# zprodev/zlib.es

Measured on AMD Instinct MI355X. Metric: GiB/s deflate+inflate round trip, 64 MiB buffers (uncompressed bytes / wall), bit-exact vs reference, higher is better.
Workload: dtype u8; 1 GPU; random64: 1 x 64 MiB xorshift buffer(s) per GPU (seed 12345+index), deflate then inflate, HBM-resident; bytes_per_buffer=67108864, compressed_bytes=67176156, parallelism=independent buffers, one per GPU

## Files before the change

include/zes.h:

```cpp
#ifndef ZES_H
#define ZES_H

#include <stdint.h>

#ifdef __cplusplus
extern "C" {
#endif

typedef enum zes_status {
  ZES_OK = 0,
  ZES_E_NOT_DEFLATE = -1,
  ZES_E_BTYPE3 = -2,
  ZES_E_CORRUPT = -3,
  ZES_E_INSUFFICIENT = -4,
  ZES_E_LACK = -5,
  ZES_E_NOSPACE = -16,
  ZES_E_DEVICE = -17,
  ZES_E_ARG = -18,
  ZES_E_NOTRANGE = -19,
  ZES_E_GZIP = -20,
  ZES_E_CHECKSUM = -21,
  ZES_E_ZIP = -22,
  ZES_E_UNSUPPORTED = -23
} zes_status;
// ... 51 lines not shown
int zes_crc32_batch_dev(const uint8_t* d_in, const uint64_t* off, const uint64_t* len, uint32_t* crc, uint32_t count);

int zes_gzip_bound(uint64_t n, uint64_t* cap);
int zes_gzip(const uint8_t* in, uint64_t n, uint8_t* out, uint64_t cap, uint64_t* out_len);
int zes_gzip_dev(const uint8_t* d_in, uint64_t n, uint8_t* d_out, uint64_t cap, uint64_t* out_len);

#define ZES_BGZF_CHUNK 65280u
int zes_bgzip_members(uint64_t n, uint64_t* members);
int zes_bgzip_bound(uint64_t n, uint64_t* cap);
int zes_bgzip(const uint8_t* in, uint64_t n, uint8_t* out, uint64_t cap, uint64_t* out_len, uint64_t* member_off, uint32_t flags);
int zes_bgzip_dev(const uint8_t* d_in, uint64_t n, uint8_t* d_out, uint64_t cap, uint64_t* out_len, uint64_t* member_off, uint32_t flags);

int zes_gunzip(const uint8_t* in, uint64_t c, uint8_t* out, uint64_t cap, uint64_t* out_len, uint32_t flags);
int zes_gunzip_dev(const uint8_t* d_in, uint64_t c, uint8_t* d_out, uint64_t cap, uint64_t* out_len, uint32_t flags);
int zes_gunzip_alloc(const uint8_t* in, uint64_t c, zes_alloc_fn alloc, void* user, uint64_t* out_len, uint32_t flags);

int zes_bgzf_index(const uint8_t* in, uint64_t c, uint64_t* coff, uint64_t* uoff, uint64_t cap, uint64_t* members, uint32_t flags);
int zes_bgzf_index_dev(const uint8_t* d_in, uint64_t c, uint64_t* coff, uint64_t* uoff, uint64_t cap, uint64_t* members, uint32_t flags);
int zes_bgzf_read(const uint8_t* in, uint64_t c, const uint64_t* coff, const uint64_t* uoff, uint64_t members, uint64_t pos, uint64_t len,
                  uint8_t* out, uint64_t cap, uint64_t* out_len, uint32_t flags);
int zes_bgzf_read_dev(const uint8_t* d_in, uint64_t c, const uint64_t* coff, const uint64_t* uoff, uint64_t members, uint64_t pos, uint64_t len,
                      uint8_t* d_out, uint64_t cap, uint64_t* out_len, uint32_t flags);

typedef struct zes_zip_entry {
  uint64_t hdr_off;
  uint64_t name_pos;
  uint32_t csize, usize, crc;
  uint32_t name_off;
  uint16_t name_len, method, flags, pad;
} zes_zip_entry;
int zes_zip_index(const uint8_t* in, uint64_t c, zes_zip_entry* ent, uint64_t cap, uint64_t* entries, uint8_t* names, uint64_t names_cap,
                  uint64_t* names_len, uint32_t flags);
int zes_zip_index_dev(const uint8_t* d_in, uint64_t c, zes_zip_entry* ent, uint64_t cap, uint64_t* entries, uint8_t* names, uint64_t names_cap,
                      uint64_t* names_len, uint32_t flags);

int zes_zip_read_dev(const uint8_t* d_in, uint64_t c, const zes_zip_entry* ent, uint64_t nent, const uint32_t* sel, uint32_t count,
                     uint8_t* d_out, const uint64_t* out_off, uint64_t* out_len, int32_t* status, uint32_t flags);
int zes_zip_read_alloc(const uint8_t* in, uint64_t c, const zes_zip_entry* ent, uint64_t nent, const uint32_t* sel, uint32_t count,
                       zes_alloc_fn alloc, void* user, uint64_t* out_len, int32_t* status, uint32_t flags);

int zes_zipwrite_bound(const uint64_t* in_len, const uint16_t* name_len, uint32_t count, uint64_t* cap);
int zes_zipwrite_dev(const uint8_t* d_in, const uint64_t* in_off, const uint64_t* in_len, const uint8_t* names, const uint16_t* name_len,
                     uint32_t count, uint8_t* d_out, uint64_t cap, uint64_t* out_len, zes_zip_entry* ent, uint32_t flags);
int zes_zipwrite(const uint8_t* const* in, const uint64_t* in_len, const uint8_t* names, const uint16_t* name_len, uint32_t count,
                 uint8_t* out, uint64_t cap, uint64_t* out_len, zes_zip_entry* ent, uint32_t flags);

int zes_adler32(const uint8_t* in, uint64_t n, uint32_t* adler);
int zes_adler32_dev(const uint8_t* d_in, uint64_t n, uint32_t* adler);
int zes_adler32_batch_dev(const uint8_t* d_in, const uint64_t* off, const uint64_t* len, uint32_t* adler, uint32_t count);

int zes_deflate_batch_dev(const uint8_t* d_in, const uint64_t* in_off, const uint64_t* in_len,
                          uint8_t* d_out, const uint64_t* out_off, const uint64_t* out_cap,
                          uint64_t* out_len, int32_t* status, uint32_t count);
int zes_inflate_batch_dev(const uint8_t* d_in, const uint64_t* in_off, const uint64_t* in_len,
                          uint8_t* d_out, const uint64_t* out_off, const uint64_t* out_cap,
                          uint64_t* out_len, int32_t* status, uint32_t count, uint32_t flags);
int zes_deflate_batch(const uint8_t* const* in, const uint64_t* in_len, uint8_t* const* out, const uint64_t* out_cap,
                      uint64_t* out_len, int32_t* status, uint32_t count);
int zes_inflate_batch_alloc(const uint8_t* const* in, const uint64_t* in_len, zes_alloc_fn alloc, void* user,
                            uint64_t* out_len, int32_t* status, uint32_t count, uint32_t flags);

int zes_deflate_range_dev(const uint8_t* d_in, uint64_t n, uint64_t n_readable, int final_range, uint8_t* d_out, uint64_t cap,
                          uint64_t* out_bits, uint32_t* adler);
int zes_deflate_join_dev(const uint8_t* const* d_piece, const uint64_t* piece_bits, const uint32_t* piece_adler,
                         const uint64_t* piece_len, uint32_t count, uint8_t* d_out, uint64_t cap, uint64_t* out_len);

int zes_inflate_range_dev(const uint8_t* d_in, uint64_t c, uint64_t lo_bit, uint64_t own_bit, int exact_start, uint8_t* d_out,
                          uint64_t cap, uint64_t* out_len, uint64_t* first_bit, uint64_t* end_bit, uint32_t* nblocks, int* final_block);

int zes_stage_lz77_dev(const uint8_t* d_in, uint64_t n, uint64_t start, uint32_t len,
                       uint32_t* h_tokens, uint32_t* ntokens);
int zes_stage_lz77_route(uint32_t* words, uint32_t cap);
int zes_stage_huff_lengths_dev(const uint32_t* h_hist, uint32_t nsym, uint32_t maxlen, uint8_t* h_lens);
int zes_stage_chain(const uint32_t* start_bit, const uint64_t* end_bit, const uint32_t* out_len, const uint32_t* flags, uint32_t count,
                    uint32_t cap, uint32_t first_bit, int on_device, int32_t* status, uint64_t* total, uint32_t* aux, uint32_t* map);

int zes_stage_poison(uint32_t word, uint64_t* bytes);

int zes_selftest_lds_order(uint32_t iters, uint32_t seed, uint64_t* bad, uint64_t* checked);

typedef struct zes_ktime { const char* name; float ms; uint32_t launches; } zes_ktime;
int zes_last_kernel_times(zes_ktime* out, int cap);
int zes_last_inflate_tier(void);
int zes_last_gunzip_members(void);
int zes_set_profiling(int on);

int zes_gen(uint8_t* out, uint64_t n, uint32_t kind, uint32_t seed);

#ifdef __cplusplus
}
#endif
#endif
```

zlib.es_amd/__init__.py:

```python
import ctypes as C
import os
import subprocess

import numpy as np

_HERE = os.path.dirname(os.path.abspath(__file__))
_LIB_PATH = os.environ.get("ZES_LIB") or os.path.join(_HERE, "libzes_hip.so")
_lib = None

BLOCK_MAX_BUFFER_LEN = 131072

ZES_OK = 0
ZES_E_NOSPACE = -16
ZES_E_DEVICE = -17
ZES_E_ARG = -18
ZES_F_NO_FASTPATH = 1
ZES_F_LOOSE_CANDIDATES = 2
ZES_F_PIECES = 4
ZES_F_ALLOC_BOUND = 8
ZES_ALLOC_EARLY = 0x80000000
ZES_E_NOTRANGE = -19
ZES_E_GZIP = -20
ZES_E_CHECKSUM = -21
ZES_E_ZIP = -22
ZES_E_UNSUPPORTED = -23
ZES_F_GZIP_SERIAL = 32
ZES_F_INDEX_WALK = 64
ZES_F_CHECK_ADLER = 16

GEN_KINDS = {"xorshift": 0, "lowent4k": 1, "itext": 2}


class ZlibEsError(Exception):

    def __init__(self, code, message):
        super().__init__(message)
        self.code = code


class ZesKTime(C.Structure):
    _fields_ = [("name", C.c_char_p), ("ms", C.c_float), ("launches", C.c_uint32)]


ZIP_ENTRY = np.dtype([("hdr_off", "<u8"), ("name_pos", "<u8"), ("csize", "<u4"), ("usize", "<u4"), ("crc", "<u4"), ("name_off", "<u4"),
                      ("name_len", "<u2"), ("method", "<u2"), ("flags", "<u2"), ("pad", "<u2")])
assert ZIP_ENTRY.itemsize == 40

ALLOC_FN = C.CFUNCTYPE(C.c_void_p, C.c_void_p, C.c_uint32, C.c_uint64)


def build(force=False):
    srcdir = os.path.join(_HERE, "csrc")
    if force:
        subprocess.check_call(["make", "-s", "-C", srcdir, "clean"])
    subprocess.check_call(["make", "-s", "-j4", "-C", srcdir])
    return _LIB_PATH


def lib():
    global _lib
    if _lib is None:
        if not os.path.exists(_LIB_PATH):
            raise RuntimeError(
                "zlib.es_amd: %s is missing — run `python -c 'import __graft_entry__ as g; g.build()'` "
                "(there is no CPU fallback)" % _LIB_PATH)
        L = C.CDLL(_LIB_PATH)
        u64p, u32p, i32p = C.POINTER(C.c_uint64), C.POINTER(C.c_uint32), C.POINTER(C.c_int32)
        L.zes_strerror.restype = C.c_char_p
        L.zes_strerror.argtypes = [C.c_int]
        L.zes_init.argtypes = [C.c_int]
        L.zes_init_devices.argtypes = [C.c_int]
        L.zes_partition.argtypes = [C.POINTER(C.c_uint64), C.c_uint32, C.c_uint32, C.POINTER(C.c_uint32)]
        L.zes_device_info.argtypes = [C.c_char_p, C.c_int, C.POINTER(C.c_int), u64p]
        L.zes_deflate_bound.argtypes = [C.c_uint64, u64p]
        for name in ("zes_deflate", "zes_deflate_dev"):
            getattr(L, name).argtypes = [C.c_void_p, C.c_uint64, C.c_void_p, C.c_uint64, u64p]
        for name in ("zes_inflate", "zes_inflate_dev"):
            getattr(L, name).argtypes = [C.c_void_p, C.c_uint64, C.c_void_p, C.c_uint64, u64p, C.c_uint32]
        L.zes_inflate_size.argtypes = [C.c_void_p, C.c_uint64, u64p, C.c_uint32]
        L.zes_inflate_alloc.argtypes = [C.c_void_p, C.c_uint64, ALLOC_FN, C.c_void_p, u64p, C.c_uint32]
        L.zes_deflate_batch.argtypes = [C.POINTER(C.c_void_p), u64p, C.POINTER(C.c_void_p), u64p, u64p, i32p, C.c_uint32]
        L.zes_inflate_batch_alloc.argtypes = [C.POINTER(C.c_void_p), u64p, ALLOC_FN, C.c_void_p, u64p, i32p, C.c_uint32, C.c_uint32]
        L.zes_host_alloc.argtypes = [C.c_uint64, C.POINTER(C.c_void_p)]
        L.zes_host_free.argtypes = [C.c_void_p]
        for name in ("zes_deflate_raw", "zes_deflate_raw_dev"):
            getattr(L, name).argtypes = [C.c_void_p, C.c_uint64, C.c_void_p, C.c_uint64, u64p]
        for name in ("zes_inflate_raw", "zes_inflate_raw_dev"):
            getattr(L, name).argtypes = [C.c_void_p, C.c_uint64, C.c_uint64, C.c_void_p, C.c_uint64, u64p, C.c_uint32]
        for name in ("zes_inflate_raw_used", "zes_inflate_raw_used_dev"):
            getattr(L, name).argtypes = [C.c_void_p, C.c_uint64, C.c_uint64, C.c_void_p, C.c_uint64, u64p, u64p, C.c_uint32]
        for name in ("zes_crc32", "zes_crc32_dev"):
            getattr(L, name).argtypes = [C.c_void_p, C.c_uint64, u32p]
        L.zes_crc32_batch_dev.argtypes = [C.c_void_p, u64p, u64p, u32p, C.c_uint32]
        L.zes_last_gunzip_members.argtypes = []
        L.zes_gzip_bound.argtypes = [C.c_uint64, u64p]
        for name in ("zes_gzip", "zes_gzip_dev"):
            getattr(L, name).argtypes = [C.c_void_p, C.c_uint64, C.c_void_p, C.c_uint64, u64p]
        for name in ("zes_gunzip", "zes_gunzip_dev"):
            getattr(L, name).argtypes = [C.c_void_p, C.c_uint64, C.c_void_p, C.c_uint64, u64p, C.c_uint32]
        for name in ("zes_bgzip_members", "zes_bgzip_bound"):
            getattr(L, name).argtypes = [C.c_uint64, u64p]
        for name in ("zes_bgzip", "zes_bgzip_dev"):
            getattr(L, name).argtypes = [C.c_void_p, C.c_uint64, C.c_void_p, C.c_uint64, u64p, u64p, C.c_uint32]
        for name in ("zes_bgzf_index", "zes_bgzf_index_dev"):
            getattr(L, name).argtypes = [C.c_void_p, C.c_uint64, C.c_void_p, C.c_void_p, C.c_uint64, u64p, C.c_uint32]
        for name in ("zes_bgzf_read", "zes_bgzf_read_dev"):
            getattr(L, name).argtypes = [C.c_void_p, C.c_uint64, C.c_void_p, C.c_void_p, C.c_uint64, C.c_uint64, C.c_uint64, C.c_void_p, C.c_uint64,
                                         u64p, C.c_uint32]
        for name in ("zes_zip_index", "zes_zip_index_dev"):
            getattr(L, name).argtypes = [C.c_void_p, C.c_uint64, C.c_void_p, C.c_uint64, u64p, C.c_void_p, C.c_uint64, u64p, C.c_uint32]
        L.zes_zip_read_dev.argtypes = [C.c_void_p, C.c_uint64, C.c_void_p, C.c_uint64, C.c_void_p, C.c_uint32, C.c_void_p, C.c_void_p, C.c_void_p,
                                       C.c_void_p, C.c_uint32]
        L.zes_zip_read_alloc.argtypes = [C.c_void_p, C.c_uint64, C.c_void_p, C.c_uint64, C.c_void_p, C.c_uint32, ALLOC_FN, C.c_void_p, C.c_void_p,
                                         C.c_void_p, C.c_uint32]
        L.zes_zipwrite_bound.argtypes = [C.c_void_p, C.c_void_p, C.c_uint32, u64p]
        L.zes_zipwrite_dev.argtypes = [C.c_void_p, C.c_void_p, C.c_void_p, C.c_void_p, C.c_void_p, C.c_uint32, C.c_void_p, C.c_uint64, u64p, C.c_void_p,
                                       C.c_uint32]
        L.zes_zipwrite.argtypes = [C.c_void_p, C.c_void_p, C.c_void_p, C.c_void_p, C.c_uint32, C.c_void_p, C.c_uint64, u64p, C.c_void_p, C.c_uint32]
        L.zes_gunzip_alloc.argtypes = [C.c_void_p, C.c_uint64, ALLOC_FN, C.c_void_p, u64p, C.c_uint32]
        L.zes_adler32.argtypes = [C.c_void_p, C.c_uint64, u32p]
        L.zes_adler32_dev.argtypes = [C.c_void_p, C.c_uint64, u32p]
        L.zes_adler32_batch_dev.argtypes = [C.c_void_p, u64p, u64p, u32p, C.c_uint32]
        L.zes_deflate_batch_dev.argtypes = [C.c_void_p, u64p, u64p, C.c_void_p, u64p, u64p, u64p, i32p, C.c_uint32]
        L.zes_inflate_batch_dev.argtypes = [C.c_void_p, u64p, u64p, C.c_void_p, u64p, u64p, u64p, i32p, C.c_uint32,
                                            C.c_uint32]
        L.zes_deflate_range_dev.argtypes = [C.c_void_p, C.c_uint64, C.c_uint64, C.c_int, C.c_void_p, C.c_uint64, u64p, u32p]
        L.zes_inflate_range_dev.argtypes = [C.c_void_p, C.c_uint64, C.c_uint64, C.c_uint64, C.c_int, C.c_void_p, C.c_uint64, u64p, u64p, u64p,
                                            u32p, i32p]
        L.zes_deflate_join_dev.argtypes = [C.POINTER(C.c_void_p), u64p, u32p, u64p, C.c_uint32, C.c_void_p, C.c_uint64, u64p]
        L.zes_stage_lz77_dev.argtypes = [C.c_void_p, C.c_uint64, C.c_uint64, C.c_uint32, C.c_void_p, u32p]
        L.zes_stage_lz77_route.argtypes = [C.c_void_p, C.c_uint32]
        L.zes_stage_huff_lengths_dev.argtypes = [C.c_void_p, C.c_uint32, C.c_uint32, C.c_void_p]
        L.zes_stage_chain.argtypes = [u32p, u64p, u32p, u32p, C.c_uint32, C.c_uint32, C.c_uint32, C.c_int, i32p, u64p, u32p, u32p]
        L.zes_stage_poison.argtypes = [C.c_uint32, u64p]
        L.zes_selftest_lds_order.argtypes = [C.c_uint32, C.c_uint32, u64p, u64p]
        L.zes_last_kernel_times.argtypes = [C.POINTER(ZesKTime), C.c_int]
        L.zes_set_profiling.argtypes = [C.c_int]
        L.zes_pool_bytes.restype = C.c_uint64
        L.zes_pool_bytes.argtypes = []
        L.zes_gen.argtypes = [C.c_void_p, C.c_uint64, C.c_uint32, C.c_uint32]
        _lib = L
    return _lib


def strerror(code):
    return lib().zes_strerror(code).decode()


def _raise(code):
    raise ZlibEsError(code, strerror(code))


def _raise_need(rc, n):
    if rc == ZES_E_NOSPACE:
        err = ZlibEsError(rc, "%s (need %d bytes)" % (strerror(rc), n.value))
        err.need = n.value
        raise err
    if rc:
        _raise(rc)


def init(device=0):
    rc = lib().zes_init(int(device))
    if rc:
        _raise(rc)


def trim():
    rc = lib().zes_trim()
    if rc:
        _raise(rc)


def pool_bytes():
    return int(lib().zes_pool_bytes())


# ... 582 lines not shown


def _batch_call(fn, d_in, in_off, in_len, d_out, out_off, out_cap, *extra):
    import torch

    cnt = len(in_off)
    arr = lambda v: (C.c_uint64 * cnt)(*[int(x) for x in v])
    out_len = (C.c_uint64 * cnt)()
    status = (C.c_int32 * cnt)()
    torch.cuda.current_stream(d_in.device).synchronize()
    rc = fn(d_in.data_ptr(), arr(in_off), arr(in_len), d_out.data_ptr(), arr(out_off), arr(out_cap), out_len, status, cnt, *extra)
    if rc:
        _raise(rc)
    return list(out_len), list(status)


def deflate_batch_tensor(d_in, in_off, in_len, d_out, out_off, out_cap):
    return _batch_call(lib().zes_deflate_batch_dev, d_in, in_off, in_len, d_out, out_off, out_cap)


def inflate_batch_tensor(d_in, in_off, in_len, d_out, out_off, out_cap, flags=0):
    return _batch_call(lib().zes_inflate_batch_dev, d_in, in_off, in_len, d_out, out_off, out_cap, flags)


def deflate_range_tensor(t, lo, hi, final, out=None):
    import torch

    assert t.is_cuda and t.dtype == torch.uint8 and t.is_contiguous() and lo % BLOCK_MAX_BUFFER_LEN == 0
    view = _aligned(t[lo:])
    n = hi - lo
    cap = deflate_bound(n)
    if out is None:
        out = torch.empty(cap, dtype=torch.uint8, device=t.device)
    torch.cuda.current_stream(t.device).synchronize()
    bits, ad = C.c_uint64(), C.c_uint32()
    rc = lib().zes_deflate_range_dev(view.data_ptr(), n, min(view.numel(), n + 258), 1 if final else 0, out.data_ptr(), out.numel(),
                                     C.byref(bits), C.byref(ad))
    if rc:
        _raise(rc)
    return out[: (bits.value + 7) // 8], bits.value, ad.value


def deflate_join_tensors(pieces, bits, adlers, lens, out=None):
    import torch

    cnt = len(pieces)
    total = 2 + (sum(bits) + 7) // 8 + 4
    if out is None:
        out = torch.empty((total + 15) // 16 * 16, dtype=torch.uint8, device=pieces[0].device)
    torch.cuda.current_stream(out.device).synchronize()
    n = C.c_uint64()
    rc = lib().zes_deflate_join_dev((C.c_void_p * cnt)(*[p.data_ptr() for p in pieces]), (C.c_uint64 * cnt)(*bits),
                                    (C.c_uint32 * cnt)(*adlers), (C.c_uint64 * cnt)(*lens), cnt, out.data_ptr(), out.numel(), C.byref(n))
    if rc:
        _raise(rc)
    return out[: n.value]


def inflate_range_tensor(t, lo_bit, own_bit, exact, out):
    import torch

    assert t.is_cuda and t.dtype == torch.uint8 and t.is_contiguous() and out.is_cuda
    lo_bit = max(16, int(lo_bit))
    byte0 = (lo_bit >> 3) & ~15
    if byte0 >= 16:
        byte0 -= 16
    end = min(t.numel(), (int(own_bit) + 7) // 8 + (1 << 20))
    view = _aligned(t[byte0:end])
    torch.cuda.current_stream(t.device).synchronize()
    n, fb, eb, nb, fin = C.c_uint64(), C.c_uint64(), C.c_uint64(), C.c_uint32(), C.c_int32()
    rc = lib().zes_inflate_range_dev(view.data_ptr(), view.numel(), lo_bit - 8 * byte0, int(own_bit) - 8 * byte0, 1 if exact else 0,
                                     out.data_ptr(), out.numel(), C.byref(n), C.byref(fb), C.byref(eb), C.byref(nb), C.byref(fin))
    if rc == ZES_E_NOTRANGE:
        return None
    if rc:
        _raise(rc)
    return n.value, fb.value + 8 * byte0, eb.value + 8 * byte0, nb.value, bool(fin.value)


def last_inflate_tier():
    return int(lib().zes_last_inflate_tier())


def last_gunzip_members():
    return int(lib().zes_last_gunzip_members())


def set_profiling(on):
    lib().zes_set_profiling(1 if on else 0)


def last_kernel_times():
    arr = (ZesKTime * 64)()
    n = lib().zes_last_kernel_times(arr, 64)
    return [(arr[i].name.decode(), float(arr[i].ms), int(arr[i].launches)) for i in range(n)]


def stage_lz77_tensor(t, start, length):
    tok = np.empty(length + 4, dtype=np.uint32)
    nt = C.c_uint32()
    rc = lib().zes_stage_lz77_dev(t.data_ptr(), t.numel(), start, length, tok.ctypes.data, C.byref(nt))
    if rc:
        _raise(rc)
    return tok[: nt.value].copy()


def stage_lz77_route():
    w = np.zeros(9, dtype=np.uint32)
    rc = lib().zes_stage_lz77_route(w.ctypes.data, w.size)
    if rc:
        _raise(rc)
    return w


def stage_poison(word):
    n = C.c_uint64(0)
    rc = lib().zes_stage_poison(int(word) & 0xFFFFFFFF, C.byref(n))
    if rc:
        _raise(rc)
    return int(n.value)


def selftest_lds_order(iters=200, seed=1):
    bad, n = C.c_uint64(0), C.c_uint64(0)
    rc = lib().zes_selftest_lds_order(iters, seed, C.byref(bad), C.byref(n))
    if rc:
        _raise(rc)
    return int(bad.value), int(n.value)


def stage_huff_lengths(hist, maxlen):
    h = np.ascontiguousarray(hist, dtype=np.uint32)
    lens = np.zeros(h.size, dtype=np.uint8)
    rc = lib().zes_stage_huff_lengths_dev(h.ctypes.data, h.size, maxlen, lens.ctypes.data)
    if rc:
        _raise(rc)
    return lens


def stage_chain(records, cap, first_bit=16, on_device=False):
    n = len(records)
    cols = [np.ascontiguousarray([r[i] for r in records], dtype=dt) for i, dt in enumerate((np.uint32, np.uint64, np.uint32, np.uint32))]
    chain = np.zeros(max(n, 1), dtype=np.uint32)
    status, total, aux = C.c_int32(), C.c_uint64(), C.c_uint32()
    u64p, u32p = C.POINTER(C.c_uint64), C.POINTER(C.c_uint32)
    ptr = lambda a, t: a.ctypes.data_as(t) if n else None
    rc = lib().zes_stage_chain(ptr(cols[0], u32p), ptr(cols[1], u64p), ptr(cols[2], u32p), ptr(cols[3], u32p), n, int(cap), int(first_bit),
                               1 if on_device else 0, C.byref(status), C.byref(total), C.byref(aux), chain.ctypes.data_as(u32p))
    if rc:
        _raise(rc)
    return int(status.value), int(total.value), int(aux.value), [int(x) for x in chain[: aux.value]] if status.value != 1 else []
```

zlib.es_amd/csrc/zes_api.hip:

```cpp
#include "../../include/zes.h"
#include "zes_kernels.h"
#include "zes_chain.h"

#include <algorithm>
#include <atomic>
#include <condition_variable>
#include <cstdio>
#include <cstddef>
#include <cstdlib>
#include <cstring>
#include <chrono>
#include <functional>
#include <future>
#include <initializer_list>
#include <map>
#include <mutex>
#include <string>
#include <thread>
#include <vector>

extern "C" int zes_gen(uint8_t* out, uint64_t n, uint32_t kind, uint32_t seed);

namespace {

// ... 71 lines not shown
    for (const PinSpan* b = a + 1; b != s.end(); ++b)
      if (a->off < b->off + b->len && b->off < a->off + a->len) return false;
  return true;
}
#define PIN_SPAN(m) PinSpan{offsetof(PinnedArea, m), sizeof(PinnedArea::m)}
#define PIN_HOLDS(m, n) static_assert(sizeof(PinnedArea::m) >= (n), #m " is smaller than its largest user")
static_assert(sizeof(PinnedArea) <= PINNED_BYTES, "the page-locked area does not fit its allocation");
PIN_HOLDS(def.res, sizeof(ZesRes) * DEFLATE_DIRECT_BUFS);
PIN_HOLDS(def.table, sizeof(ZesBuf) * DEFLATE_TABLE_BUFS);
PIN_HOLDS(t1.counters, t1_cnt_bytes(INF_GROUP));
PIN_HOLDS(t1.res, sizeof(ZesRes) * INF_GROUP);
PIN_HOLDS(t1.table, sizeof(ZesInfBuf) * (INF_GROUP + 1));
PIN_HOLDS(t1.redo, sizeof(ZesInfBuf) * 2);
PIN_HOLDS(t1.ends, sizeof(uint64_t) * 2 * INF_GROUP);
PIN_HOLDS(first.bytes, INF_GROUP);
PIN_HOLDS(first.offs, sizeof(uint64_t) * INF_GROUP);
PIN_HOLDS(t2.search, sizeof(ZesInfBuf) * (SEG_GROUP_BUFS + 1));
PIN_HOLDS(t2.ncand, sizeof(uint32_t) * SEG_GROUP_BUFS);
PIN_HOLDS(t2.flags, sizeof(uint32_t) * (SEG_GROUP_BUFS + 1));
PIN_HOLDS(t2.res, sizeof(ZesRes) * 2 * SEG_GROUP_BUFS);
PIN_HOLDS(t2.jobs, sizeof(ZesSegJob) * SEG_GROUP_BUFS);
PIN_HOLDS(t2.live, sizeof(uint32_t) * (SEG_GROUP_BUFS + 1));
PIN_HOLDS(t2.out, sizeof(ZesSegOut) * SEG_GROUP_BUFS);
PIN_HOLDS(range[0].counters, t1_cnt_bytes(1));
PIN_HOLDS(range[0].res, sizeof(ZesRes) * 2);
static_assert(sizeof(ParMirror::cres) >= sizeof(ZesCandRes) * MIRROR_ITEMS, "the mirror is smaller than its launch bound");
static_assert(sizeof(ParMirror::start) >= sizeof(uint32_t) * MIRROR_ITEMS, "the mirror is smaller than its launch bound");
static_assert(disjoint({PIN_SPAN(range[0]), PIN_SPAN(range[1])}), "the two range slots overlap");
static_assert(disjoint({PIN_SPAN(def.res), PIN_SPAN(def.table), PIN_SPAN(crc)}), "deflate regions overlap (gzip_core: the CRC words beside the results)");
static_assert(disjoint({PIN_SPAN(t1.counters), PIN_SPAN(t1.res), PIN_SPAN(t1.table), PIN_SPAN(t1.redo), PIN_SPAN(t1.ends)}), "T1 regions overlap");
static_assert(disjoint({PIN_SPAN(first.bytes), PIN_SPAN(first.offs)}), "first-byte regions overlap");
static_assert(disjoint({PIN_SPAN(t2.search), PIN_SPAN(t2.ncand), PIN_SPAN(t2.nsurv), PIN_SPAN(t2.flags), PIN_SPAN(t2.far), PIN_SPAN(t2.res),
                        PIN_SPAN(t2.jobs), PIN_SPAN(t2.live), PIN_SPAN(t2.out)}),
              "T2 regions overlap");

#define ZES_POOLS(X)                                                                                                              \
                                                                                                             \
  X(bufs) X(blks) X(idx_a) X(idx_b) X(sdelta) X(tmask) X(mlist) X(hists) X(codes) X(hdrs) X(adler) X(res) X(order)                \
                                                                                                             \
  X(surv) X(vlong) X(segfail) X(symoff) X(cand) X(cand_sorted) X(counters) X(cres) X(map) X(resume) X(dbg) X(ibufs) X(ibufs2)     \
  X(mvlist) X(scratch) X(sres) X(maps) X(seglist) X(segprefix) X(wins) X(sym16) X(segorder) X(segjobs) X(pw16) X(gwins)           \
  X(seglive) X(segouts)                                                                                                           \
                                                                                            \
  X(st_in) X(st_out)                                                                                                              \
       \
          \
        \
            \
            \
                                                                        \
  X(crctab) X(crcacc) X(gz_in) X(gz_acc) X(gz_stage) X(gz_bodies) X(gz_outs) X(gz_tab) X(crcseg)                                  \
                  \
  X(adlerseg)

struct SurvList {
  bool ok = false;
  const uint8_t* d_in = nullptr;
  uint64_t in_off = 0, c = 0;
  uint32_t n = 0, gen = 0;
  void note(const DevBuf& list, const uint8_t* din, uint64_t off, uint64_t len, uint32_t nsurv) {
    ok = true, d_in = din, in_off = off, c = len, n = nsurv, gen = list.gen;
  }
  bool holds(const DevBuf& list, const uint8_t* din, uint64_t off, uint64_t len) const {
    return ok && gen == list.gen && list.p != nullptr && d_in == din && in_off == off && c == len;
  }
  void drop() { ok = false; }
};

struct Ctx {
  bool ready = false;
  int device = -1;
  int want = -1;
  hipStream_t stream = nullptr;
  hipStream_t cs_in = nullptr, cs_out = nullptr;
  hipEvent_t ev_up[2] = {nullptr, nullptr}, ev_k = nullptr;
  hipEvent_t ev_rng[2] = {nullptr, nullptr};
  hipStream_t s_adler = nullptr;
  hipEvent_t ev_a0 = nullptr, ev_a1 = nullptr;
#define X(name) DevBuf name;
  ZES_POOLS(X)
#undef X
  uint32_t crc_npow = 0;
  DevBuf kraft;
  PinnedArea* pinned = nullptr;
  PinnedArea* pinned_dev = nullptr;
  ParMirror* mirror = nullptr;
  ParMirror* mirror_dev = nullptr;
  ZesRes* res_more = nullptr;
  size_t res_more_n = 0;
  bool profiling = false;
  std::vector<std::pair<std::string, std::pair<hipEvent_t, hipEvent_t>>> pending;
  std::vector<hipEvent_t> event_pool;
  std::vector<std::pair<std::string, KTime>> last_times;
  std::vector<std::pair<std::string, KTime>> carry;
  std::vector<std::string> name_pool;
  int last_tier = 0;
  int last_members = 0;
  uint32_t route[ZES_ROUTE_WORDS] = {0};
  SurvList sv;
  char arch[64] = {0};
  int cus = 0;
  uint64_t hbm = 0;
};
template <class F>
void for_each_pool(Ctx& c, F fn) {
#define X(name) fn(c.name);
  ZES_POOLS(X)
#undef X
}

constexpr int ZES_MAX_DEV = 16;
Ctx g_ctx[ZES_MAX_DEV];
std::mutex g_mus[ZES_MAX_DEV];
std::atomic<int> g_nctx{1};
std::mutex g_cfg_mu;
thread_local int t_dev = 0;
thread_local bool t_routed = false;
thread_local int t_last = 0;
#define g (g_ctx[t_dev])
#define g_mu (g_mus[t_dev])
struct UseDev {
  int prev;
  bool prev_routed;
  explicit UseDev(int d) : prev(t_dev), prev_routed(t_routed) {
    if (!t_routed) t_dev = d;
    t_routed = true;
    t_last = t_dev;
  }
  ~UseDev() {
    t_dev = prev;
    t_routed = prev_routed;
  }
};

#define HIPCHK(x)                                                                              \
  do {                                                                                         \
    hipError_t e_ = (x);                                                                       \
    if (e_ != hipSuccess) {                                                                    \
      if (getenv("ZES_DEBUG")) fprintf(stderr, "zes: %s failed: %s (%s:%d)\n", #x, hipGetErrorString(e_), __FILE__, __LINE__); \
      return ZES_E_DEVICE;                                                                     \
    }                                                                                          \
  } while (0)

hipError_t release(DevBuf& b) {
  const hipError_t e = b.p ? hipFree(b.p) : hipSuccess;
  b.p = nullptr;
  b.cap = 0;
  b.gen++;
  return e;
}

int ensure(DevBuf& b, size_t bytes) {
  if (bytes <= b.cap) return ZES_OK;
  HIPCHK(release(b));
  size_t want = bytes + bytes / 8 + 4096;
  HIPCHK(hipMalloc(&b.p, want));
  b.cap = want;
  return ZES_OK;
}

int init_locked(int device) {
  if (g.ready) {
    if (device >= 0 && device != g.device) return ZES_E_ARG;
    HIPCHK(hipSetDevice(g.device));
    return ZES_OK;
  }
  int n = 0;
  if (hipGetDeviceCount(&n) != hipSuccess || n <= 0) return ZES_E_DEVICE;
  if (device < 0) device = g.want >= 0 ? g.want : 0;
  if (device >= n) return ZES_E_DEVICE;
  HIPCHK(hipSetDevice(device));
  hipDeviceProp_t prop;
  HIPCHK(hipGetDeviceProperties(&prop, device));
  snprintf(g.arch, sizeof g.arch, "%s", prop.gcnArchName);
  g.cus = prop.multiProcessorCount;
  g.hbm = prop.totalGlobalMem;
  HIPCHK(hipStreamCreateWithFlags(&g.stream, hipStreamNonBlocking));
  HIPCHK(hipStreamCreateWithFlags(&g.cs_in, hipStreamNonBlocking));
  HIPCHK(hipStreamCreateWithFlags(&g.cs_out, hipStreamNonBlocking));
  for (int k = 0; k < 2; k++) HIPCHK(hipEventCreateWithFlags(&g.ev_up[k], hipEventDisableTiming));
  for (int k = 0; k < 2; k++) HIPCHK(hipEventCreateWithFlags(&g.ev_rng[k], hipEventDisableTiming));
  HIPCHK(hipEventCreateWithFlags(&g.ev_k, hipEventDisableTiming));
  HIPCHK(hipStreamCreateWithFlags(&g.s_adler, hipStreamNonBlocking));
  HIPCHK(hipEventCreateWithFlags(&g.ev_a0, hipEventDisableTiming));
  HIPCHK(hipEventCreateWithFlags(&g.ev_a1, hipEventDisableTiming));
  auto dev_addr = [](void* h) -> void* {
    void* d = nullptr;
    if (hipHostGetDevicePointer(&d, h, 0) == hipSuccess) return d;
    (void)hipGetLastError();
    return nullptr;
  };
  HIPCHK(hipHostMalloc((void**)&g.pinned, PINNED_BYTES, hipHostMallocDefault));
  g.pinned_dev = (PinnedArea*)dev_addr(g.pinned);
  if (hipHostMalloc((void**)&g.mirror, sizeof(ParMirror), hipHostMallocDefault) == hipSuccess) {
    g.mirror_dev = (ParMirror*)dev_addr(g.mirror);
  } else {
    (void)hipGetLastError();
    g.mirror = nullptr;
  }
  {
    uint8_t tab[4096];
    for (uint32_t i = 0; i < 4096; i++) {
      uint32_t k = 0;
      for (uint32_t f = 0; f < 4; f++) k += (128u >> ((i >> (3 * f)) & 7u)) & 127u;
      tab[i] = (uint8_t)std::min(k, 200u);
    }
    HIPCHK(hipMalloc(&g.kraft.p, 4096));
    g.kraft.cap = 4096;
    HIPCHK(hipMemcpy(g.kraft.p, tab, 4096, hipMemcpyHostToDevice));
  }
  g.device = device;
  g.ready = true;
  return ZES_OK;
}

int route_host() {
  if (t_routed) return t_dev;
  const int n = g_nctx.load();
  if (n <= 1) return 0;
  static std::atomic<uint32_t> rr{0};
  return (int)(rr.fetch_add(1) % (uint32_t)n);
}
int route_dev(const void* p, const void* p2 = nullptr) {
  if (t_routed) return t_dev;
  if (g_nctx.load() <= 1 || !p) return 0;
  hipPointerAttribute_t a;
  if (hipPointerGetAttributes(&a, p) != hipSuccess) {
    (void)hipGetLastError();
    return -1;
  }
  if (p2) {
    hipPointerAttribute_t b;
    if (hipPointerGetAttributes(&b, p2) != hipSuccess) {
      (void)hipGetLastError();
      return -1;
    }
    if (b.device != a.device) return -1;
  }
  for (int i = 0, n = g_nctx.load(); i < n; i++)
    if ((g_ctx[i].ready ? g_ctx[i].device : g_ctx[i].want) == a.device) return i;
  return -1;
}
#define ROUTE_DEV(...)                    \
  const int rd_ = route_dev(__VA_ARGS__); \
  if (rd_ < 0) return ZES_E_ARG;          \
  UseDev ud(rd_)
#define LOCK_READY()                    \
  std::lock_guard<std::mutex> lk(g_mu); \
  int rc = init_locked(-1);             \
  if (rc) return rc

constexpr size_t STAGE_CHUNK = 8u << 20;
constexpr int STAGE_RING = 4;
constexpr size_t STAGE_DIRECT_MAX = 256u << 10;

struct CopyPool {
  std::vector<std::thread> threads;
  std::mutex mu;
  std::condition_variable cv_work, cv_done;
  uint8_t* dst = nullptr;
  const uint8_t* src = nullptr;
  size_t n = 0, part = 0;
  uint32_t gen = 0, parts = 0;
  std::atomic<uint32_t> next{0};
  uint32_t done = 0, active = 0;
  bool stop = false;

  void worker() {
    uint32_t seen = 0;
    std::unique_lock<std::mutex> lk(mu);
    for (;;) {
      cv_work.wait(lk, [&] { return stop || gen != seen; });
      if (stop) return;
      seen = gen;
      active++;
      lk.unlock();
      const uint32_t did = run_parts();
      lk.lock();
      done += did;
      active--;
      if (done >= parts && active == 0) cv_done.notify_all();
    }
  }
  uint32_t run_parts() {
    uint32_t did = 0;
    for (;;) {
      const uint32_t k = next.fetch_add(1);
      if (k >= parts) return did;
      const size_t o = (size_t)k * part;
      memcpy(dst + o, src + o, std::min(part, n - o));
      did++;
    }
  }
// ... 646 lines not shown

int t1_pools(uint32_t nbuf, uint32_t surv_cap, uint64_t cands, size_t counter_bytes, uint32_t nres) {
  int rc;
  if ((rc = ensure(g.ibufs, sizeof(ZesInfBuf) * (nbuf + 1)))) return rc;
  if ((rc = ensure(g.surv, (size_t)surv_cap * 8))) return rc;
  if ((rc = ensure(g.cand, (size_t)cands * 4))) return rc;
  if ((rc = ensure(g.cand_sorted, (size_t)cands * 4))) return rc;
  if ((rc = ensure(g.cres, sizeof(ZesCandRes) * cands))) return rc;
  if ((rc = ensure(g.counters, counter_bytes))) return rc;
  return ensure(g.res, sizeof(ZesRes) * nres);
}

ZesRes t1_host_chain(const uint32_t* start, const ZesCandRes* cres, const uint32_t* hc, uint32_t surv_cap, const ZesInfBuf& b, uint64_t work,
                     uint32_t* map) {
  const ZesChainView v = {start, cres, std::min(hc[4], b.cand_cap), 0u};
  const uint32_t nwork = hc[0] != 0 && hc[0] <= surv_cap ? (uint32_t)std::min<uint64_t>(v.n, work) : 0u;
  return zes_chain_decide(v, hc[4], b.cand_cap, nwork, 16u + (uint64_t)b.start_rel, map);
}

struct T1Group {
  const uint8_t* d_in;
  uint8_t* d_out;
  InfJob* jobs;
  const uint32_t* ids;
  uint32_t nbuf, flags;
  bool check_first, one;
  ZesInfBuf* hb;
  uint32_t* hc;
  ZesRes* hres;
  uint64_t chunks = 0, cands = 0, total_c = 0, work = 0;
  uint32_t surv_cap = 0;
  size_t cnt_bytes = 0;
  const ZesInfBuf* dbufs = nullptr;
  uint32_t *counters = nullptr, *cnt = nullptr;
  unsigned long long* dbg = nullptr;
  bool hostchain = false;
  std::vector<uint32_t> ncand;
  std::vector<ZesRes> r1;
};
constexpr int T1_OVER = 1;

bool t1_first_byte(T1Group& t, uint32_t i, uint8_t fb) {
  InfJob& j = t.jobs[t.ids[i]];
  if (fb & 0x40u) j.btype0 = (fb >> 4) & 3;
  if (!t.check_first || (fb & 15u) == 8u) return false;
  j.status = ZES_E_NOT_DEFLATE;
  j.tier = -1;
  return true;
}

int t1_table(T1Group& t) {
  int rc;
  g.sv.drop();
  ZesInfBuf* hb = t.hb;
  for (uint32_t i = 0; i < t.nbuf; i++) {
    const InfJob& j = t.jobs[t.ids[i]];
    ZesInfBuf& b = hb[i] = inf_buf(j);
    b.first_chunk = (uint32_t)t.chunks;
    b.cand_base = (uint32_t)t.cands;
    b.cand_cap = (uint32_t)std::min<uint64_t>(j.c / 64 + 64, j.cap / ZES_BLK + 65);
    b.own_rel = 0xFFFFFFFFu;
    t.chunks += (j.c + INF_SCAN_BYTES - 1) / INF_SCAN_BYTES;
    t.cands += b.cand_cap;
    t.total_c += j.c;
  }
  if (t.chunks >= (1ull << 31) || t.cands >= (1ull << 31)) return T1_OVER;
  const uint32_t nbuf = t.nbuf;
  memset(&hb[nbuf], 0, sizeof(ZesInfBuf));
  hb[nbuf].first_chunk = (uint32_t)t.chunks;
  hb[nbuf].cand_base = (uint32_t)t.cands;
  if (t.one) {
    hb[1].work_first = ZES_WORK_AUTO;
    hb[1].cand_cap = hb[0].cand_cap;
  }
  t.surv_cap = (uint32_t)std::min<uint64_t>(t.total_c / 4 + 1024ull * nbuf, 1ull << 30);
  t.cnt_bytes = t1_cnt_bytes(nbuf);
  if ((rc = t1_pools(nbuf, t.surv_cap, t.cands, t.cnt_bytes, nbuf))) return rc;
  if ((rc = ensure(g.map, (size_t)t.cands * 4))) return rc;
  t.dbufs = (const ZesInfBuf*)g.ibufs.p;
  t.counters = (uint32_t*)g.counters.p;
  t.cnt = t.counters + 4;
  if (t.one) {
    hipLaunchKernelGGL(k_inf_set_table1, dim3(1), dim3(64), 0, g.stream, hb[0], hb[1], (ZesInfBuf*)g.ibufs.p, t.counters,
                       (uint32_t)(t.cnt_bytes / 4));
  } else {
    HIPCHK(hipMemcpyAsync(g.ibufs.p, hb, sizeof(ZesInfBuf) * (nbuf + 1), hipMemcpyHostToDevice, g.stream));
    HIPCHK(hipMemsetAsync(g.counters.p, 0, t.cnt_bytes, g.stream));
  }
  return ZES_OK;
}

int t1_decode(T1Group& t) {
  int rc;
  const uint32_t nbuf = t.nbuf;
  ZesInfBuf* hb = t.hb;
  uint32_t* hc = t.hc;
  if (!t.one) {
    HIPCHK(hipMemcpyAsync(hc, g.counters.p, t.cnt_bytes, hipMemcpyDeviceToHost, g.stream));
    HIPCHK(hipStreamSynchronize(g.stream));
    const uint8_t* hfirst = (const uint8_t*)(hc + 4 + nbuf);
    for (uint32_t i = 0; i < nbuf; i++)
      if (t1_first_byte(t, i, hfirst[i])) hc[4 + i] = 0;
    const uint32_t nsurv0 = hc[0];
    if (nsurv0 != 0 && nsurv0 <= t.surv_cap)
      for (uint32_t i = 0; i < nbuf; i++) {
        t.ncand[i] = hc[4 + i];
        hb[i].work_first = (uint32_t)t.work;
        if (t.ncand[i] > 0 && t.ncand[i] <= hb[i].cand_cap) t.work += t.ncand[i];
      }
    hb[nbuf].work_first = (uint32_t)t.work;
    if (t.work == 0) return T1_OVER;
    HIPCHK(hipMemcpyAsync(g.ibufs.p, hb, sizeof(ZesInfBuf) * (nbuf + 1), hipMemcpyHostToDevice, g.stream));
  } else {
    t.work = hb[1].cand_cap;
  }
  if (getenv("ZES_DEBUG_PHASES")) {
    if ((rc = ensure(g.dbg, (size_t)t.work * ZES_PAR_DBG_ROW * 8))) return rc;
    HIPCHK(hipMemsetAsync(g.dbg.p, 0, (size_t)t.work * ZES_PAR_DBG_ROW * 8, g.stream));
    t.dbg = (unsigned long long*)g.dbg.p;
  }
  uint64_t total_cap = 0;
  for (uint32_t i = 0; i < nbuf; i++) total_cap += t.jobs[t.ids[i]].cap;
  const bool two = t.total_c * 10 < total_cap * 7;
  ZesParMirror mir{};
  if (t.one && t.work <= MIRROR_ITEMS && g.mirror_dev && g.pinned_dev) {
    mir.cres_host = g.mirror_dev->cres;
    mir.start_host = g.mirror_dev->start;
    mir.counters = t.counters;
    mir.counters_host = g.pinned_dev->t1.counters;
    mir.counter_words = (uint32_t)(t.cnt_bytes / 4);
    t.hostchain = true;
  }
  launch_block_par(two ? "k_inf_block_par2" : "k_inf_block_par", two, (uint32_t)t.work, t.d_in, t.d_out, t.dbufs, nbuf, t.cnt, t.dbg, nullptr, mir);
  return ZES_OK;
}

int t1_device_chain(T1Group& t) {
  Timed tm("k_inf_chain");
  const bool direct = t.one && g.pinned_dev;
  hipLaunchKernelGGL(k_inf_chain, dim3(t.nbuf), dim3(256), 0, g.stream, t.dbufs, (const uint32_t*)t.cnt, (const uint32_t*)g.cand_sorted.p,
                     (const ZesCandRes*)g.cres.p, (const uint32_t*)nullptr, (uint32_t*)g.map.p,
                     direct ? g.pinned_dev->t1.res : (ZesRes*)g.res.p, (const uint32_t*)t.counters, (uint32_t)(t.cnt_bytes / 4),
                     direct ? g.pinned_dev->t1.counters : (uint32_t*)nullptr);
  if (!direct) {
    if (t.one) HIPCHK(hipMemcpyAsync(t.hc, g.counters.p, t.cnt_bytes, hipMemcpyDeviceToHost, g.stream));
    HIPCHK(hipMemcpyAsync(t.hres, g.res.p, sizeof(ZesRes) * t.nbuf, hipMemcpyDeviceToHost, g.stream));
  }
  return ZES_OK;
}

int t1_verdicts(T1Group& t) {
  int rc;
  uint32_t* hc = t.hc;
  if (!t.hostchain && (rc = t1_device_chain(t))) return rc;
  host_lap("(work before the block-parallel tier)");
  HIPCHK(hipStreamSynchronize(g.stream));
  host_lap("T1: search + decode + chain");
  if (t.hostchain) {
    ZesRes r = t1_host_chain(g.mirror->start, g.mirror->cres, hc, t.surv_cap, t.hb[0], t.work, nullptr);
    if (r.status == 2) {
      if ((rc = t1_device_chain(t))) return rc;
      HIPCHK(hipStreamSynchronize(g.stream));
      r = t.hres[0];
    } else {
      t.hres[0] = r;
    }
    if (getenv("ZES_DEBUG")) {
      const ZesCandRes* hcr = g.mirror->cres;
      const uint32_t* hst = g.mirror->start;
      fprintf(stderr, "zes T1 host chain: nsurv %u cnt %u cap %u work %llu -> status %d out_len %llu | start0 %u", hc[0], hc[4], t.hb[0].cand_cap,
              (unsigned long long)t.work, r.status, (unsigned long long)r.out_len, hst[0]);
      for (uint32_t k = 0; k < std::min<uint32_t>(hc[4], 10u); k++)
        fprintf(stderr, " [%u: start %u end %llu len %u fl %u]", k, hst[k], (unsigned long long)hcr[k].end_bit, hcr[k].out_len, hcr[k].flags);
      fprintf(stderr, "\n");
    }
  }
  const uint32_t nsurv = hc[0];
  if (t.one) {
    const InfJob& j = t.jobs[t.ids[0]];
    if (t1_first_byte(t, 0, ((const uint8_t*)(hc + 5))[0])) return T1_OVER;
    t.ncand[0] = hc[4];
    if (nsurv != 0 && nsurv <= t.surv_cap && !(t.flags & ZES_F_LOOSE_CANDIDATES))
      g.sv.note(g.surv, t.d_in, j.in_off, j.c, nsurv);
    if (nsurv == 0 || nsurv > t.surv_cap || t.ncand[0] == 0 || t.ncand[0] > t.hb[0].cand_cap || t.ncand[0] > t.work) return T1_OVER;
    t.hb[0].work_first = 0;
    t.work = t.ncand[0];
  }
  t.r1.assign(t.hres, t.hres + t.nbuf);
  if (t.dbg && (rc = print_par_phases(t.dbg, t.work))) return rc;
  if (getenv("ZES_DEBUG")) {
    for (uint32_t i = 0, shown_b = 0; i < t.nbuf && shown_b < 4; i++) {
      const ZesRes& r = t.r1[i];
      if (r.status == 0) continue;
      shown_b++;
      const uint32_t nc = std::min(t.ncand[i], t.hb[i].cand_cap);
      fprintf(stderr, "zes T1: buf %u c=%llu nsurv(all)=%u ncand=%u chain status=%d aux=%u out_len=%llu\n", t.ids[i],
              (unsigned long long)t.hb[i].c, nsurv, t.ncand[i], r.status, r.aux, (unsigned long long)r.out_len);
      if (r.status != 1 || nc == 0) continue;
      std::vector<ZesCandRes> hcr(nc);
      std::vector<uint32_t> hcand(nc);
      HIPCHK(hipMemcpy(hcr.data(), (const ZesCandRes*)g.cres.p + t.hb[i].cand_base, sizeof(ZesCandRes) * nc, hipMemcpyDeviceToHost));
      HIPCHK(hipMemcpy(hcand.data(), (const uint32_t*)g.cand_sorted.p + t.hb[i].cand_base, 4 * (size_t)nc, hipMemcpyDeviceToHost));
      const ZesChainView v = {hcand.data(), hcr.data(), nc, 16u};
      int shown = 0;
      for (uint32_t k = 0; k < nc && shown < 6; k++) {
        if (k + 1 < nc ? zes_chain_link(v, hcr[k], k + 1) : (hcr[k].flags & ZES_CAND_OK) != 0) continue;
        fprintf(stderr, "  cand %u start=%u end_bit=%llu next_start=%u out_len=%u flags=%u\n", k, (uint32_t)zes_chain_start(v, k),
                (unsigned long long)hcr[k].end_bit, k + 1 < nc ? (uint32_t)zes_chain_start(v, k + 1) : 0, hcr[k].out_len, hcr[k].flags);
        shown++;
      }
    }
  }
  return ZES_OK;
}

// ... 640 lines not shown
  G.ccap.resize(nb);
  G.searched.assign(nb, 0);
  uint64_t cands = 0, max_c = 0;
  for (uint32_t k = 0; k < nb; k++) {
    const InfJob& j = G.jobs[G.ids[k]];
    G.cbase[k] = (uint32_t)cands;
    G.ccap[k] = range_cand_cap(j.c);
    cands += G.ccap[k];
    max_c = std::max(max_c, j.c);
  }
  G.surv_cap = range_surv_cap(max_c);
  G.w = seg_words(nb, nb);
  if ((rc = ensure(g.ibufs, sizeof(ZesInfBuf) * 2))) return rc;
  if ((rc = ensure(g.surv, (size_t)G.surv_cap * 8))) return rc;
  if ((rc = ensure(g.cand, (size_t)cands * 4))) return rc;
  if ((rc = ensure(g.cand_sorted, (size_t)cands * 4))) return rc;
  if ((rc = ensure(g.counters, G.w.total * 4))) return rc;
  if ((rc = ensure(g.mvlist, SEG_BUCKETS * 4))) return rc;
  G.counters = (uint32_t*)g.counters.p + G.w.scan;
  G.cnt = (uint32_t*)g.counters.p + G.w.cnt;
  G.sink = (uint8_t*)((uint32_t*)g.counters.p + G.w.sink);
  HIPCHK(hipMemsetAsync(g.counters.p, 0, G.w.total * 4, g.stream));
  G.dbufs = (const ZesInfBuf*)g.ibufs.p;
  return ZES_OK;
}

ZesInfBuf t2_search_buf(const T2Group& G, uint32_t k) {
  const InfJob& j = G.jobs[G.ids[k]];
  ZesInfBuf b = inf_buf(j);
  b.cand_base = G.cbase[k];
  b.cand_cap = G.ccap[k];
  b.start_rel = j.start0 - 16u;
  return b;
}

int t2_search_group(T2Group& G) {
  int rc;
  const uint32_t nb = G.nb;
  ZesInfBuf* hb = g.pinned->t2.search;
  uint64_t chunks = 0, total_c = 0;
  for (uint32_t k = 0; k < nb; k++) {
    hb[k] = t2_search_buf(G, k);
    hb[k].first_chunk = (uint32_t)chunks;
    chunks += (hb[k].c + INF_SCAN_BYTES - 1) / INF_SCAN_BYTES;
    total_c += hb[k].c;
  }
  memset(&hb[nb], 0, sizeof(ZesInfBuf));
  hb[nb].first_chunk = (uint32_t)chunks;
  const uint32_t surv_all = (uint32_t)std::min<uint64_t>(total_c / 4 + 1024ull * nb, 1ull << 30);
  if ((rc = ensure(g.ibufs, sizeof(ZesInfBuf) * (nb + 1)))) return rc;
  if ((rc = ensure(g.surv, (size_t)surv_all * 8))) return rc;
  G.dbufs = (const ZesInfBuf*)g.ibufs.p;
  HIPCHK(hipMemcpyAsync(g.ibufs.p, hb, sizeof(ZesInfBuf) * (nb + 1), hipMemcpyHostToDevice, g.stream));
  if ((rc = launch_search(G.d_in, G.dbufs, nb, (uint32_t)chunks, surv_all, G.counters, G.cnt, G.sink, T2_SEARCH, total_c))) return rc;
  {
    Timed t("k_inf_ranksort");
    hipLaunchKernelGGL(k_inf_ranksort, dim3(nb), dim3(1024), 0, g.stream, G.dbufs, (const uint32_t*)G.cnt, (const uint32_t*)g.cand.p,
                       (uint32_t*)g.cand_sorted.p, SEG_BUCKETS);
  }
  uint32_t* hc0 = g.pinned->t2.ncand;
  HIPCHK(hipMemcpyAsync(hc0, G.cnt, (size_t)nb * 4, hipMemcpyDeviceToHost, g.stream));
  HIPCHK(hipStreamSynchronize(g.stream));
  bool redo = false;
  for (uint32_t k = 0; k < nb; k++) {
    G.searched[k] = hc0[k] <= SEG_BUCKETS;
    redo = redo || !G.searched[k];
  }
  if (redo) {
    if ((rc = ensure(g.ibufs2, sizeof(ZesInfBuf) * 2))) return rc;
    G.dbufs = (const ZesInfBuf*)g.ibufs2.p;
  }
  return ZES_OK;
}

int t2_search_one(T2Group& G, uint32_t k) {
  int rc;
  uint32_t* cntk = G.cnt + k;
  HIPCHK(hipMemsetAsync(cntk, 0, 4, g.stream));
  const ZesInfBuf b0 = t2_search_buf(G, k);
  const uint32_t chunks = (uint32_t)((b0.c + INF_SCAN_BYTES - 1) / INF_SCAN_BYTES);
  ZesInfBuf b1;
  memset(&b1, 0, sizeof b1);
  b1.first_chunk = chunks;
  hipLaunchKernelGGL(k_inf_set_table1, dim3(1), dim3(64), 0, g.stream, b0, b1, const_cast<ZesInfBuf*>(G.dbufs), G.counters, 4u);
  const bool reuse = G.nb == 1 && g.sv.holds(g.surv, G.d_in, b0.in_off, b0.c) && b0.start_rel == 0u && g.sv.n <= G.surv_cap;
  g.sv.drop();
  if (reuse) {
    g.pinned->t2.nsurv = g.sv.n;
    HIPCHK(hipMemcpyAsync(G.counters, &g.pinned->t2.nsurv, 4, hipMemcpyHostToDevice, g.stream));
    rc = launch_verify(G.d_in, G.dbufs, G.surv_cap, G.counters, cntk, T2_SEARCH.loose, b0.c);
  } else {
    rc = launch_search(G.d_in, G.dbufs, 1u, chunks, G.surv_cap, G.counters, cntk, G.sink, T2_SEARCH, b0.c);
  }
  if (rc) return rc;
  Timed t("k_inf_cand_thin");
  const uint32_t bucket_bits = (uint32_t)((b0.c * 8 + SEG_BUCKETS - 1) / SEG_BUCKETS);
  HIPCHK(hipMemsetAsync(g.mvlist.p, 0xFF, SEG_BUCKETS * 4, g.stream));
  hipLaunchKernelGGL(k_inf_cand_bucket, dim3((uint32_t)std::min<uint64_t>(b0.cand_cap / 256 + 1, 1024)), dim3(256), 0, g.stream,
                     (const uint32_t*)g.cand.p + b0.cand_base, (const uint32_t*)cntk, b0.cand_cap, bucket_bits, (uint32_t*)g.mvlist.p);
  hipLaunchKernelGGL(k_inf_cand_compact, dim3(1), dim3(1024), 0, g.stream, (const uint32_t*)g.mvlist.p,
                     (uint32_t*)g.cand_sorted.p + b0.cand_base, cntk);
  return ZES_OK;
}

int t2_group_counts(T2Group& G) {
  const uint32_t nb = G.nb;
  uint32_t* hc = g.pinned->t2.ncand;
  HIPCHK(hipMemcpyAsync(hc, G.cnt, (size_t)nb * 4, hipMemcpyDeviceToHost, g.stream));
  host_lap("(host work since)");
  HIPCHK(hipStreamSynchronize(g.stream));
  host_lap("T2: search (verify, thinning)");
  G.nc.assign(hc, hc + nb);
  if (getenv("ZES_T2_DBG")) {
    for (uint32_t k = 0; k < nb; k++) {
      std::vector<uint32_t> hcand(std::min<uint32_t>(G.nc[k], SEG_BUCKETS));
      if (!hcand.empty()) HIPCHK(hipMemcpy(hcand.data(), (const uint32_t*)g.cand_sorted.p + G.cbase[k], hcand.size() * 4, hipMemcpyDeviceToHost));
      fprintf(stderr, "zes T2 candidates buf %u (%zu):", k, hcand.size());
      for (uint32_t v : hcand) fprintf(stderr, " %u", v + 16u);
      fprintf(stderr, "\n");
    }
  }
  return ZES_OK;
}

int t2_group_runs(T2Group& G) {
  int rc;
  std::vector<uint32_t> rid, rbase, rn;
  for (uint32_t k = 0; k < G.nb;) {
    uint32_t work = 0;
    rid.clear();
    rbase.clear();
    rn.clear();
    for (; k < G.nb; k++) {
      if (G.nc[k] > SEG_BUCKETS) continue;
      if (!rid.empty() && work + G.nc[k] + 1 > SEG_GROUP_WORK) break;
      rid.push_back(G.ids[k]);
      rbase.push_back(G.cbase[k]);
      rn.push_back(G.nc[k]);
      work += G.nc[k] + 1;
    }
    const uint32_t nr = (uint32_t)rid.size();
    if (nr && (rc = inflate_segments_run(G.d_in, G.d_out, G.jobs, rid.data(), rbase.data(), rn.data(), nr, seg_words(G.nb, nr)))) return rc;
  }
  return ZES_OK;
}

int inflate_segments(const uint8_t* d_in, uint8_t* d_out, InfJob* jobs, const std::vector<uint32_t>& all) {
  int rc;
  for (size_t g0 = 0; g0 < all.size(); g0 += SEG_GROUP_BUFS) {
    T2Group G{d_in, d_out, jobs, all.data() + g0, (uint32_t)std::min<size_t>(SEG_GROUP_BUFS, all.size() - g0)};
    if ((rc = t2_group_table(G))) return rc;
    if (G.nb > 1 && (rc = t2_search_group(G))) return rc;
    for (uint32_t k = 0; k < G.nb; k++)
      if (!G.searched[k] && (rc = t2_search_one(G, k))) return rc;
    if ((rc = t2_group_counts(G))) return rc;
    if ((rc = t2_group_runs(G))) return rc;
  }
  return ZES_OK;
}

constexpr uint64_t STORED_MIN_C = 65536;
int inflate_segments_pieces(const uint8_t* d_in, uint8_t* d_out, InfJob& j) {
  static const uint64_t piece = [] {
    const char* e = getenv("ZES_SEG_PIECE_MB");
    const uint64_t mb = e ? strtoull(e, nullptr, 10) : 0;
    return mb ? (mb << 20) : (32ull << 20);
  }();
// ... 19 lines not shown
    }
    if (sub[0].tier != 2) return ZES_OK;
    piece_now = piece;
    if (sub[0].status == ZES_E_NOSPACE) nospace = true;
    else if (sub[0].status != ZES_OK) return ZES_OK;
    out_base += sub[0].out_len;
    if (sub[0].final_seen) {
      j.tier = 2;
      j.status = (nospace || out_base > j.cap) ? ZES_E_NOSPACE : ZES_OK;
      j.out_len = out_base;
      j.end_bit = 8 * byte0 + sub[0].end_bit;
      return ZES_OK;
    }
    const uint64_t next_bit = 8 * byte0 + sub[0].end_bit;
    if (!sub[0].partial || next_bit <= pos_bit) return ZES_OK;
    pos_bit = next_bit;
  }
  return ZES_OK;
}

int inflate_stored(const uint8_t* d_in, uint8_t* d_out, InfJob& j) {
  int rc;
  const uint64_t cap_entries = std::min<uint64_t>(j.c / 5 + 1, 1ull << 22);
  if ((rc = ensure(g.res, sizeof(ZesRes)))) return rc;
  if ((rc = ensure(g.scratch, (size_t)cap_entries * sizeof(ZesStoredBlk)))) return rc;
  ZesRes hr;
  hr.status = 1;
  constexpr uint64_t STORED_PAR_MAX_C = 128ull << 20;
  constexpr uint32_t STORED_CHUNK_H = 16384, STORED_SLOTS_H = 8;
  if (j.c >= (2ull << 20) && j.c <= STORED_PAR_MAX_C && !getenv("ZES_NO_STORED_PAR")) {
    const uint32_t nchunks = (uint32_t)((j.c + STORED_CHUNK_H - 1) / STORED_CHUNK_H);
    if ((rc = ensure(g.mvlist, (size_t)nchunks * (STORED_SLOTS_H + 1) * 4))) return rc;
    uint32_t* slots = (uint32_t*)g.mvlist.p;
    uint32_t* counts = slots + (size_t)nchunks * STORED_SLOTS_H;
    {
      Timed t("k_inf_stored_find");
      hipLaunchKernelGGL(k_inf_stored_find, dim3(nchunks), dim3(256), 0, g.stream, d_in, j.in_off, (uint32_t)j.c, slots, counts);
    }
    {
      Timed t("k_inf_stored_rank");
      hipLaunchKernelGGL(k_inf_stored_rank, dim3(1), dim3(1024), 0, g.stream, d_in, j.in_off, (uint32_t)j.c, (const uint32_t*)slots,
                         (const uint32_t*)counts, nchunks, cap_entries, (ZesStoredBlk*)g.scratch.p, (ZesRes*)g.res.p);
    }
    if ((rc = read_res(&hr))) return rc;
  }
  if (hr.status != 0) {
    Timed t("k_inf_stored_walk");
    hipLaunchKernelGGL(k_inf_stored_walk, dim3(1), dim3(64), 0, g.stream, d_in, j.in_off, j.c, cap_entries, (ZesStoredBlk*)g.scratch.p,
                       (ZesRes*)g.res.p);
    if ((rc = read_res(&hr))) return rc;
  }
  if (hr.status != 0) return ZES_OK;
  j.tier = 2;
  j.out_len = hr.out_len;
  j.status = hr.out_len > j.cap ? ZES_E_NOSPACE : ZES_OK;
  if (j.want_end && hr.aux) {
    ZesStoredBlk last;
    HIPCHK(hipMemcpy(&last, (const ZesStoredBlk*)g.scratch.p + hr.aux - 1, sizeof last, hipMemcpyDeviceToHost));
    j.end_bit = 8 * (last.src + last.len);
  }
  if (j.status == ZES_OK && hr.aux) {
    Timed t("k_inf_stored_copy");
    hipLaunchKernelGGL(k_inf_stored_copy, dim3(hr.aux), dim3(256), 0, g.stream, d_in, j.in_off, d_out, j.out_off, (const ZesStoredBlk*)g.scratch.p);
    HIPCHK(hipStreamSynchronize(g.stream));
  }
  return ZES_OK;
}

int inflate_slow(const uint8_t* d_in, uint8_t* d_out, InfJob& j) {
  int rc;
  if ((rc = ensure(g.res, 2 * sizeof(ZesRes)))) return rc;
  if ((rc = ensure(g.resume, 16))) return rc;
  ZesRes hr;
  bool have_resume = false;
  if (j.c >= 3) {
#ifdef WD_PROFILE
    if ((rc = ensure(g.dbg, 64))) return rc;
    HIPCHK(hipMemsetAsync(g.dbg.p, 0, 64, g.stream));
    zes_wd_set_dbg((unsigned long long*)g.dbg.p);
#endif
    {
      const ZesInfBuf b0 = inf_buf(j);
      if ((rc = ensure(g.ibufs, sizeof(ZesInfBuf) * 2))) return rc;
      hipLaunchKernelGGL(k_inf_set_table1, dim3(1), dim3(64), 0, g.stream, b0, b0, (ZesInfBuf*)g.ibufs.p, (uint32_t*)nullptr, 0u);
      Timed t("k_inf_decode_seq");
      hipLaunchKernelGGL(k_inf_decode, dim3(1), dim3(64), 0, g.stream, d_in, d_out, (const ZesInfBuf*)g.ibufs.p, (ZesRes*)g.res.p,
                         (uint64_t*)g.resume.p);
    }
    if ((rc = read_res(&hr))) return rc;
#ifdef WD_PROFILE
    {
      unsigned long long h[8];
      HIPCHK(hipMemcpy(h, g.dbg.p, 64, hipMemcpyDeviceToHost));
      const double n = (double)std::max<unsigned long long>(h[5], 1);
      fprintf(stderr, "zes wave decoder: %llu tokens, cycles per token: lit/len entry %.1f, literal path %.1f, distance entry %.1f, copy %.1f, flush test %.1f; kernel %.1f\n",
              h[5], h[0] / n, h[1] / n, h[2] / n, h[3] / n, h[4] / n, h[6] / n);
    }
#endif
    if (hr.status == 0) {
      j.tier = 3;
      j.out_len = hr.out_len;
      j.status = hr.out_len > j.cap ? ZES_E_NOSPACE : ZES_OK;
      if (j.want_end) HIPCHK(hipMemcpy(&j.end_bit, g.resume.p, 8, hipMemcpyDeviceToHost));
      return ZES_OK;
    }
    have_resume = true;
  }
  {
    Timed t("k_inf_exact");
    hipLaunchKernelGGL(k_inf_exact, dim3(1), dim3(64), 0, g.stream, d_in, j.in_off, j.c, d_out, j.out_off, j.cap,
                       have_resume ? (const uint64_t*)g.resume.p : (const uint64_t*)nullptr, (ZesRes*)g.res.p);
  }
  if ((rc = read_res(&hr))) return rc;
  if (j.want_end) {
    ZesRes r2;
    HIPCHK(hipMemcpy(&r2, (const ZesRes*)g.res.p + 1, sizeof r2, hipMemcpyDeviceToHost));
    j.end_bit = r2.out_len;
  }
  j.tier = 4;
  j.out_len = hr.out_len;
  j.status = hr.status;
  return ZES_OK;
}

constexpr uint64_t T1_PIECE = 256ull << 20;
constexpr uint64_t T1_PIECE_SLACK = 1ull << 20;
int inflate_pieces(const uint8_t* d_in, uint8_t* d_out, InfJob& j, uint32_t flags) {
  uint64_t piece = T1_PIECE;
  if (flags & ZES_F_PIECES) piece = 1ull << 20;
  uint64_t pos_bit = 16, total = 0, blocks = 0;
  for (uint32_t round = 0; round < (1u << 20); round++) {
    uint64_t byte0 = (pos_bit >> 3) & ~15ull;
    if (byte0 >= 16) byte0 -= 16;
    const uint64_t rel = pos_bit - 8 * byte0;
    const uint64_t pc = std::min<uint64_t>(j.c - byte0, piece + T1_PIECE_SLACK);
    const uint64_t done_bytes = blocks * ZES_BLK;
    RangeRes rr;
    int rc = inflate_t1_range(d_in, j.in_off + byte0, pc, rel, rel + piece * 8, true, d_out, j.out_off + std::min(done_bytes, j.cap),
                              j.cap > done_bytes ? j.cap - done_bytes : 0, flags, &rr);
    if (rc) return rc;
    if (!rr.handled || rr.nblocks == 0) return ZES_OK;
    blocks += rr.nblocks;
    total += rr.out_len;
    pos_bit = 8 * byte0 + rr.end_bit;
    if (rr.final_block) {
      j.tier = 1;
      j.out_len = total;
      j.end_bit = pos_bit;
      j.status = total > j.cap ? ZES_E_NOSPACE : ZES_OK;
      return ZES_OK;
    }
    if (pos_bit >= j.c * 8) return ZES_OK;
  }
  return ZES_OK;
}

int gather_bytes(const uint8_t* d_in, const std::vector<InfJob>& jobs, const uint32_t* ids, uint32_t nb, uint32_t at, const uint8_t** bytes) {
  int rc;
  if ((rc = ensure(g.ibufs, (size_t)INF_GROUP * 8 + INF_GROUP))) return rc;
  uint64_t* ho = g.pinned->first.offs;
  for (uint32_t k = 0; k < nb; k++) ho[k] = jobs[ids[k]].in_off + at;
  uint8_t* dfirst = (uint8_t*)g.ibufs.p + (size_t)INF_GROUP * 8;
  HIPCHK(hipMemcpyAsync(g.ibufs.p, ho, (size_t)nb * 8, hipMemcpyHostToDevice, g.stream));
  hipLaunchKernelGGL(k_inf_first_bytes, dim3((nb + 255) / 256), dim3(256), 0, g.stream, d_in, (const uint64_t*)g.ibufs.p, dfirst, nb);
  HIPCHK(hipMemcpyAsync(g.pinned->first.bytes, dfirst, nb, hipMemcpyDeviceToHost, g.stream));
  HIPCHK(hipStreamSynchronize(g.stream));
  *bytes = g.pinned->first.bytes;
// ... 286 lines not shown
    case ZES_E_CORRUPT: return "Data is corrupted";
    case ZES_E_INSUFFICIENT: return "Data length is insufficient";
    case ZES_E_LACK: return "Lack of data length";
    case ZES_E_NOSPACE: return "zes: output capacity too small";
    case ZES_E_DEVICE: return "zes: HIP device error (no gfx950 device or runtime failure)";
    case ZES_E_ARG: return "zes: bad argument";
    case ZES_E_NOTRANGE: return "zes: not a clean chain of reference-made blocks in this range";
    case ZES_E_GZIP: return "zes: not a valid gzip member (header or trailer)";
    case ZES_E_CHECKSUM: return "zes: checksum mismatch";
    case ZES_E_ZIP: return "zes: not a valid ZIP archive or entry (end record, directory or local header)";
    case ZES_E_UNSUPPORTED: return "zes: unsupported ZIP feature (ZIP64, several disks, encryption, a method other than 0 or 8)";
    default: return "zes: unknown status";
  }
}

int zes_init(int device) {
  UseDev ud(0);
  std::lock_guard<std::mutex> lk(g_mu);
  return init_locked(device);
}

int zes_init_devices(int n) {
  int have = 0;
  if (hipGetDeviceCount(&have) != hipSuccess || have <= 0) return ZES_E_DEVICE;
  const bool over = getenv("ZES_OVERSUBSCRIBE") != nullptr;
  if (n <= 0) n = have;
  if (n > ZES_MAX_DEV || (n > have && !over)) return ZES_E_ARG;
  std::lock_guard<std::mutex> cfg(g_cfg_mu);
  for (int i = 0; i < n; i++) {
    std::lock_guard<std::mutex> lk(g_mus[i]);
    const int dev = i % have;
    if (g_ctx[i].ready ? g_ctx[i].device != dev : (g_ctx[i].want >= 0 && g_ctx[i].want != dev)) return ZES_E_ARG;
    g_ctx[i].want = dev;
  }
  if (n > g_nctx.load()) g_nctx.store(n);
  for (int i = 0; i < n; i++) {
    UseDev ud(i);
    LOCK_READY();
  }
  return ZES_OK;
}

static int shutdown_one(void);
int zes_shutdown(void) {
  std::lock_guard<std::mutex> cfg(g_cfg_mu);
  int rc = ZES_OK;
  for (int i = 0; i < ZES_MAX_DEV; i++) {
    t_dev = i;
    const int r = shutdown_one();
    if (r && !rc) rc = r;
    g_ctx[i].want = -1;
  }
  t_dev = 0;
  g_nctx.store(1);
  return rc;
}

static void free_scratch_locked() {
  for_each_pool(g, [](DevBuf& b) { (void)release(b); });
}

int zes_trim(void) {
  std::lock_guard<std::mutex> cfg(g_cfg_mu);
  const int keep = t_dev;
  for (int i = 0; i < ZES_MAX_DEV; i++) {
    t_dev = i;
    std::lock_guard<std::mutex> lk(g_mu);
    if (!g.ready) continue;
    (void)hipSetDevice(g.device);
    (void)hipStreamSynchronize(g.stream);
    free_scratch_locked();
  }
  t_dev = keep;
  return ZES_OK;
}

static int shutdown_one(void) {
  std::lock_guard<std::mutex> lk(g_mu);
  if (!g.ready) return ZES_OK;
  (void)hipSetDevice(g.device);
  (void)hipStreamSynchronize(g.stream);
  free_scratch_locked();
  (void)release(g.kraft);
  if (g.pinned) (void)hipHostFree(g.pinned);
  if (g.mirror) (void)hipHostFree(g.mirror);
  if (g.res_more) (void)hipHostFree(g.res_more);
  g.pinned = g.pinned_dev = nullptr;
  g.mirror = g.mirror_dev = nullptr;
  g.res_more = nullptr;
  g.res_more_n = 0;
  g_side_up.shutdown();
  g_side_down.shutdown();
  g_up.release();
  g_down.release();
  for (hipEvent_t e : g.event_pool) (void)hipEventDestroy(e);
  g.event_pool.clear();
  (void)hipStreamDestroy(g.stream);
  (void)hipStreamDestroy(g.cs_in);
  (void)hipStreamDestroy(g.cs_out);
  for (int k = 0; k < 2; k++) (void)hipEventDestroy(g.ev_up[k]);
  for (int k = 0; k < 2; k++) (void)hipEventDestroy(g.ev_rng[k]);
  (void)hipEventDestroy(g.ev_k);
  (void)hipStreamDestroy(g.s_adler);
  (void)hipEventDestroy(g.ev_a0);
  (void)hipEventDestroy(g.ev_a1);
  g.s_adler = nullptr;
  g.stream = g.cs_in = g.cs_out = nullptr;
  g.ready = false;
  return ZES_OK;
}

int zes_host_alloc(uint64_t n, void** p) {
  UseDev ud(0);
  if (!p) return ZES_E_ARG;
  *p = nullptr;
  LOCK_READY();
  HIPCHK(hipHostMalloc(p, n ? n : 1, hipHostMallocPortable));
  return ZES_OK;
}

int zes_host_free(void* p) {
  if (!p) return ZES_OK;
  std::lock_guard<std::mutex> lk(g_mu);
  if (g.ready) (void)hipSetDevice(g.device);
  HIPCHK(hipHostFree(p));
  return ZES_OK;
}

int zes_device_info(char* name, int cap, int* cus, uint64_t* hbm_bytes) {
  LOCK_READY();
  if (name && cap > 0) snprintf(name, (size_t)cap, "%s", g.arch);
  if (cus) *cus = g.cus;
  if (hbm_bytes) *hbm_bytes = g.hbm;
  return ZES_OK;
}

int zes_deflate_bound(uint64_t n, uint64_t* cap) {
  if (!cap) return ZES_E_ARG;
  *cap = deflate_bound(n);
  return ZES_OK;
}

int zes_deflate_batch_dev(const uint8_t* d_in, const uint64_t* in_off, const uint64_t* in_len, uint8_t* d_out,
                          const uint64_t* out_off, const uint64_t* out_cap, uint64_t* out_len, int32_t* status, uint32_t count) {
  ROUTE_DEV(d_in, d_out);
  if (!in_off || !in_len || !out_off || !out_cap || !out_len || !status) return ZES_E_ARG;
  LOCK_READY();
  return deflate_batch_core(d_in, in_off, in_len, d_out, out_off, out_cap, out_len, status, count);
}

int zes_deflate_dev(const uint8_t* d_in, uint64_t n, uint8_t* d_out, uint64_t cap, uint64_t* out_len) {
  ROUTE_DEV(d_in, d_out);
  if (!out_len) return ZES_E_ARG;
  uint64_t zero = 0;
  int32_t st = 0;
  int rc = zes_deflate_batch_dev(d_in, &zero, &n, d_out, &zero, &cap, out_len, &st, 1);
  return rc ? rc : st;
}

struct SettleGuard {
  std::future<int>&a, &b;
  ~SettleGuard() {
    if (a.valid()) a.wait();
    if (b.valid()) b.wait();
  }
};
// ... 2318 lines not shown
    if ((rc = t1_pools(1, 0, (uint64_t)cap + 1, sizeof hc, 1))) return rc;
    if ((rc = ensure(g.map, (size_t)cap * 4 + 4))) return rc;
    uint32_t* counters = (uint32_t*)g.counters.p;
    HIPCHK(hipMemcpyAsync(g.ibufs.p, tab, sizeof tab, hipMemcpyHostToDevice, g.stream));
    HIPCHK(hipMemcpyAsync(counters, hc, sizeof hc, hipMemcpyHostToDevice, g.stream));
    if (n) {
      HIPCHK(hipMemcpyAsync(g.cand_sorted.p, rel.data(), (size_t)n * 4, hipMemcpyHostToDevice, g.stream));
      HIPCHK(hipMemcpyAsync(g.cres.p, cres.data(), sizeof(ZesCandRes) * n, hipMemcpyHostToDevice, g.stream));
    }
    hipLaunchKernelGGL(k_inf_chain, dim3(1), dim3(256), 0, g.stream, (const ZesInfBuf*)g.ibufs.p, (const uint32_t*)(counters + 4),
                       (const uint32_t*)g.cand_sorted.p, (const ZesCandRes*)g.cres.p, (const uint32_t*)nullptr, (uint32_t*)g.map.p, (ZesRes*)g.res.p,
                       (const uint32_t*)counters, 0u, (uint32_t*)nullptr);
    HIPCHK(hipGetLastError());
    if ((rc = read_res(&r))) return rc;
    if (r.status != 1 && r.aux <= n) HIPCHK(hipMemcpy(map, g.map.p, (size_t)r.aux * 4, hipMemcpyDeviceToHost));
  }
  *status = r.status;
  *total = r.out_len;
  *aux = r.aux;
  return ZES_OK;
}

static int poison_locked(Ctx& c, uint32_t word, uint64_t* filled) {
  HIPCHK(hipSetDevice(c.device));
  const hipStream_t streams[] = {c.stream, c.cs_in, c.cs_out, c.s_adler};
  for (hipStream_t s : streams) HIPCHK(hipStreamSynchronize(s));
  hipError_t e = hipSuccess;
  for_each_pool(c, [&](DevBuf& b) {
    const size_t words = b.p ? b.cap / 4 : 0;
    if (!words || e != hipSuccess) return;
    e = hipMemsetD32Async((hipDeviceptr_t)b.p, (int)word, words, c.stream);
    *filled += (uint64_t)words * 4;
  });
  HIPCHK(e);
  auto fill = [&](void* p, size_t bytes) {
    if (!p) return;
    std::fill((uint32_t*)p, (uint32_t*)p + bytes / 4, word);
    *filled += bytes / 4 * 4;
  };
  fill(c.pinned, PINNED_BYTES);
  fill(c.mirror, sizeof(ParMirror));
  fill(c.res_more, sizeof(ZesRes) * c.res_more_n);
  c.sv.drop();
  c.crc_npow = 0;
  HIPCHK(hipStreamSynchronize(c.stream));
  return ZES_OK;
}

int zes_stage_poison(uint32_t word, uint64_t* bytes) {
  std::lock_guard<std::mutex> cfg(g_cfg_mu);
  uint64_t filled = 0;
  int rc = ZES_OK;
  for (int i = 0; i < ZES_MAX_DEV; i++) {
    std::lock_guard<std::mutex> lk(g_mus[i]);
    if (!g_ctx[i].ready) continue;
    const int r = poison_locked(g_ctx[i], word, &filled);
    if (r && !rc) rc = r;
  }
  if (bytes) *bytes = filled;
  return rc;
}

int zes_selftest_lds_order(uint32_t iters, uint32_t seed, uint64_t* bad, uint64_t* checked) {
  if (!bad || !checked || iters == 0 || iters > 100000u) return ZES_E_ARG;
  LOCK_READY();
  if ((rc = ensure(g.hists, 320 * 4))) return rc;
  HIPCHK(hipMemsetAsync(g.hists.p, 0, 16, g.stream));
  hipLaunchKernelGGL(k_selftest_lds_order, dim3(256), dim3(SORT_THREADS), 0, g.stream, (unsigned long long*)g.hists.p, iters, seed);
  HIPCHK(hipGetLastError());
  unsigned long long h[2] = {0, 0};
  HIPCHK(hipMemcpyAsync(h, g.hists.p, 16, hipMemcpyDeviceToHost, g.stream));
  HIPCHK(hipStreamSynchronize(g.stream));
  *bad = h[0];
  *checked = h[1];
  return ZES_OK;
}

int zes_last_inflate_tier(void) {
  UseDev ud(t_last);
  std::lock_guard<std::mutex> lk(g_mu);
  return g.last_tier;
}

int zes_last_gunzip_members(void) {
  UseDev ud(t_last);
  std::lock_guard<std::mutex> lk(g_mu);
  return g.last_members;
}

int zes_set_profiling(int on) {
  std::lock_guard<std::mutex> cfg(g_cfg_mu);
  for (int i = 0; i < ZES_MAX_DEV; i++) {
    std::lock_guard<std::mutex> lk(g_mus[i]);
    g_ctx[i].profiling = on != 0;
  }
  return ZES_OK;
}

uint64_t zes_pool_bytes(void) {
  uint64_t total = 0;
  for (int i = 0; i < ZES_MAX_DEV; i++) {
    std::lock_guard<std::mutex> lk(g_mus[i]);
    for_each_pool(g_ctx[i], [&](const DevBuf& b) { total += b.cap; });
  }
  return total;
}

int zes_last_kernel_times(zes_ktime* out, int cap) {
  UseDev ud(t_last);
  std::lock_guard<std::mutex> lk(g_mu);
  int n = 0;
  g.name_pool.clear();
  for (auto& e : g.last_times) g.name_pool.push_back(e.first);
  for (size_t i = 0; i < g.last_times.size() && n < cap; i++, n++) {
    out[n].name = g.name_pool[i].c_str();
    out[n].ms = (float)g.last_times[i].second.ms;
    out[n].launches = g.last_times[i].second.launches;
  }
  return n;
}

}
```

zlib.es_amd/csrc/zes_inflate.hip:

```cpp
#include "zes_common.h"
#include "zes_kernels.h"
#include "zes_chain.h"

#define ZES_E_NOT_DEFLATE (-1)
#define ZES_E_BTYPE3 (-2)
#define ZES_E_CORRUPT (-3)
#define ZES_E_INSUFFICIENT (-4)
#define ZES_E_LACK (-5)

__device__ static inline uint64_t g_load64_le(const uint8_t* p, uint64_t byte, uint64_t nbytes) {
  uint64_t v = 0;
#pragma unroll
  for (int k = 0; k < 8; k++) {
    const uint64_t b = byte + k;
    v |= (uint64_t)(b < nbytes ? p[b] : (uint8_t)0) << (8 * k);
  }
  return v;
}

#define SCAN_BYTES INF_SCAN_BYTES
#define RANK_LDS 8192u
#define VERIFY_STEPS 32u
#define SCAN_LIST 1024u
__global__ __launch_bounds__(256) void k_inf_move_slots(uint8_t* __restrict__ dst, const uint8_t* __restrict__ src,
                                                        const uint32_t* __restrict__ dst_slot, const uint32_t* __restrict__ src_slot,
                                                        uint32_t nitems) {
  const uint32_t item = blockIdx.x >> 5, part = blockIdx.x & 31u;
  if (item >= nitems) return;
  const uint4* s4 = reinterpret_cast<const uint4*>(src + (uint64_t)src_slot[item] * ZES_BLK) + part * 256u;
  uint4* d4 = reinterpret_cast<uint4*>(dst + (uint64_t)dst_slot[item] * ZES_BLK) + part * 256u;
  d4[threadIdx.x] = s4[threadIdx.x];
}

__global__ void k_inf_set_table1(ZesInfBuf b0, ZesInfBuf sentinel, ZesInfBuf* __restrict__ bufs, uint32_t* __restrict__ counters,
                                 uint32_t nwords) {
  if (threadIdx.x == 0) {
    bufs[0] = b0;
    bufs[1] = sentinel;
  }
  if (counters && threadIdx.x < nwords) counters[threadIdx.x] = 0;
}

__global__ void k_inf_set_table_range(ZesInfBuf b0, ZesInfBuf sentinel, ZesInfBuf* __restrict__ bufs, uint32_t* __restrict__ counters,
                                      uint32_t nwords, const unsigned long long* __restrict__ acc, unsigned long long dcap) {
  if (threadIdx.x == 0) {
    const unsigned long long off = acc[0] * ZES_BLK;
    b0.out_off += off < dcap ? off : dcap;
    b0.cap = dcap - (off < dcap ? off : dcap);
    bufs[0] = b0;
    bufs[1] = sentinel;
  }
  if (counters && threadIdx.x < nwords) counters[threadIdx.x] = 0;
}

__global__ void k_inf_first_bytes(const uint8_t* __restrict__ d_in, const uint64_t* __restrict__ offs, uint8_t* __restrict__ out,
                                  uint32_t n) {
  const uint32_t i = blockIdx.x * blockDim.x + threadIdx.x;
  if (i < n) out[i] = d_in[offs[i]];
}

__device__ __forceinline__ static uint32_t buf_of_chunk(const ZesInfBuf* bufs, uint32_t nbuf, uint32_t x) {
  uint32_t lo = 0, hi = nbuf;
  while (hi - lo > 1) {
    const uint32_t mid = (lo + hi) >> 1;
    if (bufs[mid].first_chunk <= x) lo = mid; else hi = mid;
  }
  return lo;
}

#define SCAN_FINAL_ZONE_BITS (160u * 1024u * 8u)
__global__ __launch_bounds__(INF_SCAN_THREADS) void k_inf_scan(const uint8_t* __restrict__ d_in, const ZesInfBuf* __restrict__ bufs,
                                                               uint32_t nbuf, unsigned long long* __restrict__ surv,
                                                               uint32_t surv_cap, uint32_t* __restrict__ counters,
                                                               uint8_t* __restrict__ first_bytes, uint32_t mode,
                                                               const uint8_t* __restrict__ kraft_tab) {
  const uint32_t loose = mode & 1u;
  __shared__ __align__(16) uint32_t s[SCAN_BYTES / 4 + 8];
  __shared__ uint32_t s_list[SCAN_LIST];
  __shared__ uint32_t s_cnt, s_base;
  __shared__ __align__(16) uint8_t s_kraft[4096];
  const uint32_t tid = threadIdx.x;
  if (tid == 0) s_cnt = 0;
  static_assert(INF_SCAN_THREADS * 16 == 4096, "one 16-byte load per thread");
  reinterpret_cast<uint4*>(s_kraft)[tid] = reinterpret_cast<const uint4*>(kraft_tab)[tid];
  const uint32_t bi = buf_of_chunk(bufs, nbuf, blockIdx.x);
  const uint64_t in_off = bufs[bi].in_off, c = bufs[bi].c;
  const uint64_t b0 = (uint64_t)(blockIdx.x - bufs[bi].first_chunk) * SCAN_BYTES;
  const uint32_t* in32 = reinterpret_cast<const uint32_t*>(d_in + in_off);
  const uint64_t ndw = (c + 3) >> 2;
  uint32_t hdr2 = 0;
  bool hdr_known = false;
  if ((mode & 2u) && !loose && !(bufs[bi].range_flags & ZES_START_ANY)) {
    const uint64_t hbit = 16ull + bufs[bi].start_rel;
    if (hbit + 3 <= c * 8) {
      const uint64_t hb = hbit >> 3;
      hdr2 = ((uint32_t)d_in[in_off + hb] | ((uint32_t)d_in[in_off + (hb + 1 < c ? hb + 1 : hb)] << 8)) >> (uint32_t)(hbit & 7u);
      hdr_known = true;
    }
  }
  {
    constexpr uint32_t NLD = (SCAN_BYTES / 4 + 8 + INF_SCAN_THREADS - 1) / INF_SCAN_THREADS;
    uint32_t v[NLD];
#pragma unroll
    for (uint32_t j = 0; j < NLD; j++) {
      const uint64_t gi = (b0 >> 2) + tid + j * INF_SCAN_THREADS;
      v[j] = in32[gi < ndw ? gi : ndw - 1];
    }
#pragma unroll
    for (uint32_t j = 0; j < NLD; j++) {
      const uint32_t i = tid + j * INF_SCAN_THREADS;
      const uint64_t gi = (b0 >> 2) + i;
      uint32_t x = v[j];
      if (gi == ndw - 1 && (c & 3u)) x &= (1u << (8u * (uint32_t)(c & 3u))) - 1u;
      if (gi >= ndw) x = 0;
      if (i < SCAN_BYTES / 4 + 8) s[i] = x;
    }
  }
  __syncthreads();
  if (tid == 0 && b0 == 0) first_bytes[bi] = (uint8_t)((s[0] & 0x0fu) | (((s[0] >> 17) & 3u) << 4) | 0x40u);
  if (hdr_known && ((hdr2 >> 1) & 3u) != 2u) return;
  const uint64_t end_bits = c * 8;
// ... 2538 lines not shown
```

zlib.es_amd/csrc/zes_inflate_par.hip:

```cpp
#include "zes_common.h"
#include "zes_kernels.h"
#include "zes_chain.h"

#define PL_ROOT 10u
#define PD_ROOT 9u
#define F_EOB 1u
#define F_FAIL 2u
#define F_VOID 4u
#define F_HIST 8u

#define RES_W 4096u
#define P4_SPARSE_DEP_MAX 32u
#define P4_SPARSE_MAX 1024u
#ifndef RES_REPS
#define RES_REPS 4u
#endif
#define PAR_CHUNK (ZES_BLK - 3u * RES_W)
#define PAR_DIST_OFF (PAR_CHUNK + 64u)
#define PAR_MAX_OUT (1u << 27)
#define STAGE_DW ((ZES_BLK + ZES_BLK / 8) / 4)
struct ParSmem {
  uint8_t out[ZES_BLK];
  uint32_t bitmap[ZES_BLK / 32];
  uint32_t lut_l[1u << PL_ROOT];
// ... 87 lines not shown

struct Lit8 {
  uint32_t lo, n, off;
};
__device__ __forceinline__ static uint32_t lead_lit8(uint32_t w, const Lit8& f) {
  const uint32_t r = __brev(w);
  const bool a = ((r >> 24) - f.lo) < f.n, b = (((r >> 16) & 255u) - f.lo) < f.n, c = (((r >> 8) & 255u) - f.lo) < f.n,
             d = ((r & 255u) - f.lo) < f.n;
  uint32_t n = d ? 4u : 3u;
  n = c ? n : 2u;
  n = b ? n : 1u;
  n = a ? n : 0u;
  return n;
}

struct SegTab {
  uint64_t a, b, c, d, e, f, g, h;
};
__device__ __forceinline__ static uint32_t tab_get(const SegTab& t, uint32_t o) {
  const uint32_t wi = o >> 3;
  uint64_t a = t.a, b = t.b, c = t.c, d = t.d, e = t.e, f = t.f, g = t.g, h = t.h;
  asm("" : "+v"(a), "+v"(b), "+v"(c), "+v"(d));
  asm("" : "+v"(e), "+v"(f), "+v"(g), "+v"(h));
  uint64_t x = a;
  x = (wi == 1u) ? b : x;
  x = (wi == 2u) ? c : x;
  x = (wi == 3u) ? d : x;
  x = (wi == 4u) ? e : x;
  x = (wi == 5u) ? f : x;
  x = (wi == 6u) ? g : x;
  x = (wi == 7u) ? h : x;
  return (uint32_t)(x >> ((o & 7u) * 8u)) & 0xffu;
}
__device__ __forceinline__ static void tab_set(SegTab& t, uint32_t o, uint32_t code) {
  const uint32_t wi = o >> 3;
  const uint64_t v = (uint64_t)code << ((o & 7u) * 8u);
  t.a |= (wi == 0u) ? v : 0ull;
  t.b |= (wi == 1u) ? v : 0ull;
  t.c |= (wi == 2u) ? v : 0ull;
  t.d |= (wi == 3u) ? v : 0ull;
  t.e |= (wi == 4u) ? v : 0ull;
  t.f |= (wi == 5u) ? v : 0ull;
  t.g |= (wi == 6u) ? v : 0ull;
  t.h |= (wi == 7u) ? v : 0ull;
}
__device__ __forceinline__ static void tab_put(SegTab& t, uint32_t o, uint32_t code, bool doit) {
  const uint32_t wi = o >> 3, sh = (o & 7u) * 8u;
  const uint64_t m = doit ? (0xffull << sh) : 0ull, v = doit ? ((uint64_t)code << sh) : 0ull;
  t.a = (wi == 0u) ? ((t.a & ~m) | v) : t.a;
  t.b = (wi == 1u) ? ((t.b & ~m) | v) : t.b;
  t.c = (wi == 2u) ? ((t.c & ~m) | v) : t.c;
  t.d = (wi == 3u) ? ((t.d & ~m) | v) : t.d;
  t.e = (wi == 4u) ? ((t.e & ~m) | v) : t.e;
  t.f = (wi == 5u) ? ((t.f & ~m) | v) : t.f;
  t.g = (wi == 6u) ? ((t.g & ~m) | v) : t.g;
  t.h = (wi == 7u) ? ((t.h & ~m) | v) : t.h;
}
__device__ __forceinline__ static uint64_t tab_nzmask(const SegTab& t) {
  auto nz8 = [](uint64_t w) -> uint64_t {
    const uint64_t k7 = 0x7f7f7f7f7f7f7f7full;
    const uint64_t y = (((w & k7) + k7) | w) & ~k7;
    return ((y >> 7) * 0x0102040810204080ull) >> 56;
  };
  return nz8(t.a) | (nz8(t.b) << 8) | (nz8(t.c) << 16) | (nz8(t.d) << 24) | (nz8(t.e) << 32) | (nz8(t.f) << 40) | (nz8(t.g) << 48) | (nz8(t.h) << 56);
}
__device__ __forceinline__ static uint64_t bcast64(uint64_t v, uint32_t srclane) {
  const uint32_t lo = (uint32_t)__builtin_amdgcn_readlane((int)(uint32_t)v, (int)srclane);
  const uint32_t hi = (uint32_t)__builtin_amdgcn_readlane((int)(uint32_t)(v >> 32), (int)srclane);
  return (uint64_t)lo | ((uint64_t)hi << 32);
}
__device__ __forceinline__ static SegTab tab_bcast(const SegTab& t, uint32_t srclane) {
  SegTab r;
  r.a = bcast64(t.a, srclane);
  r.b = bcast64(t.b, srclane);
  r.c = bcast64(t.c, srclane);
  r.d = bcast64(t.d, srclane);
  r.e = bcast64(t.e, srclane);
  r.f = bcast64(t.f, srclane);
  r.g = bcast64(t.g, srclane);
  r.h = bcast64(t.h, srclane);
  return r;
}

__device__ __forceinline__ static int slow_sym(const LaneBits& b, uint32_t root, const uint16_t* syms, const uint32_t* first,
                                               const uint16_t* cnt, const uint16_t* offs, uint32_t* len_out) {
  uint32_t code = __brev((uint32_t)b.bb & ((1u << root) - 1u)) >> (32u - root);
  for (uint32_t len = root + 1; len <= 15u; len++) {
    code = (code << 1) | (uint32_t)((b.bb >> (len - 1)) & 1u);
    const uint32_t f = first[len];
    const uint32_t rel = code - f;
    if (code >= f && rel < cnt[len]) {
      *len_out = len;
      return (int)syms[offs[len] + rel];
    }
  }
  return -1;
}

#define T_LIT 0u
#define T_EOB 1u
#define T_MATCH 2u
#define T_FAIL 3u
#define C_EOB 62u
#define C_FAIL 63u
#define C_NONE 255u

template <bool LDS>
__device__ __forceinline__ static uint32_t tok_step(ParSmem& S, LaneBits& b, const BitSrc& src, uint32_t& val, uint32_t& len,
                                                    uint32_t& dist) {
  lb_refill<LDS>(b, src);
  uint32_t e = S.lut_l[(uint32_t)b.bb & ((1u << PL_ROOT) - 1u)];
  if ((e & 15u) == 0u) {
    uint32_t l2 = 0;
    const int sy = slow_sym(b, PL_ROOT, S.syms_l, S.first_l, S.cnt_l, S.offs_l, &l2);
    if (sy < 0) return T_FAIL;
    e = entry_l((uint32_t)sy, l2);
  }
  lb_take(b, e & 15u);
  const uint32_t kind = (e >> 8) & 3u;
  if (kind == 0u) {
    val = e >> 16;
    return T_LIT;
  }
  if (kind == 1u) return T_EOB;
  if (kind == 3u) return T_FAIL;
  lb_refill<LDS>(b, src);
  len = (e >> 16) + lb_take(b, (e >> 4) & 15u);
  lb_refill<LDS>(b, src);
  uint32_t ed = S.lut_d[(uint32_t)b.bb & ((1u << PD_ROOT) - 1u)];
  if ((ed & 15u) == 0u) {
    uint32_t l2 = 0;
    const int sy = slow_sym(b, PD_ROOT, S.syms_d, S.first_d, S.cnt_d, S.offs_d, &l2);
    if (sy < 0) return T_FAIL;
    ed = entry_d((uint32_t)sy, l2);
  }
  lb_take(b, ed & 15u);
  if (((ed >> 8) & 3u) != 2u) return T_FAIL;
  lb_refill<LDS>(b, src);
  dist = (ed >> 16) + lb_take(b, (ed >> 4) & 15u);
  return T_MATCH;
}

__device__ __forceinline__ static uint32_t lut_l_entry(ParSmem& S, uint32_t bits) {
  uint32_t e = S.lut_l[bits & ((1u << PL_ROOT) - 1u)];
  if ((e & 15u) == 0u) {
    LaneBits t;
    t.bb = bits;
    uint32_t l2 = 0;
    const int sy = slow_sym(t, PL_ROOT, S.syms_l, S.first_l, S.cnt_l, S.offs_l, &l2);
    e = sy < 0 ? 0u : entry_l((uint32_t)sy, l2);
  }
  return e;
}
__device__ __forceinline__ static uint32_t lut_d_entry(ParSmem& S, uint32_t bits) {
  uint32_t e = S.lut_d[bits & ((1u << PD_ROOT) - 1u)];
  if ((e & 15u) == 0u) {
    LaneBits t;
    t.bb = bits;
    uint32_t l2 = 0;
    const int sy = slow_sym(t, PD_ROOT, S.syms_d, S.first_d, S.cnt_d, S.offs_d, &l2);
    e = sy < 0 ? 0u : entry_d((uint32_t)sy, l2);
  }
  return e;
}

__device__ __forceinline__ static void lb_refill_bf(LaneBits& b, const BitSrc& s) {
  const bool need = b.nb <= 32u;
  const uint32_t k = ((b.pos + b.nb) >> 5) - s.s_first;
  const bool in = k < s.s_count;
  const uint32_t kk = in ? k : 0u;
  uint32_t w = s.s32[kk ^ ((kk >> 5) & 31u)];
  w = in ? w : 0u;
  const uint32_t sh = need ? b.nb : 0u;
  const uint64_t add = (uint64_t)w << sh;
  b.bb |= need ? add : 0ull;
  b.nb += need ? 32u : 0u;
}

__device__ __forceinline__ static void len_step(ParSmem& S, const BitSrc& src, LaneBits& b, bool act, uint32_t& adv, bool& eob,
                                                bool& bad) {
  lb_refill_bf(b, src);
  const uint32_t a = S.len_l[(uint32_t)b.bb & ((1u << PL_ROOT) - 1u)];
  uint32_t n = a & 63u;
  const bool sp = (a & 0x80u) != 0u;
  bool m = (a & 0x40u) != 0u;
  eob = false;
  bad = false;
  if (__ballot(act && sp)) {
    const uint32_t e = lut_l_entry(S, (uint32_t)b.bb);
    const uint32_t kind = (e >> 8) & 3u;
    if (sp) {
      eob = kind == 1u;
      bad = (kind == 3u) || ((e & 15u) == 0u);
      n = (e & 15u) + ((e >> 4) & 15u);
      m = kind == 2u;
    }
  }
  if (__ballot(act && m)) {
    LaneBits t = b;
    t.bb >>= n;
    t.nb -= n;
    t.pos += n;
    lb_refill_bf(t, src);
    const uint32_t d = S.len_d[(uint32_t)t.bb & ((1u << PD_ROOT) - 1u)];
    uint32_t n2 = d & 63u;
    const bool dsp = (d & 0x80u) != 0u;
    if (__ballot(act && m && dsp)) {
      const uint32_t ed = lut_d_entry(S, (uint32_t)t.bb);
      if (dsp) {
        bad = bad || (m && ((((ed >> 8) & 3u) != 2u) || (ed & 15u) == 0u));
        n2 = (ed & 15u) + ((ed >> 4) & 15u);
      }
    }
    if (act && m) {
      b = t;
      n = n2;
    }
  }
  adv = n;
}

#define NX_EOB 0xFEu
#define NX_FAIL 0xFFu

__device__ __forceinline__ static uint32_t win_bits(uint32_t a0, uint32_t a1, uint32_t a2, uint32_t a3, uint32_t a4, uint32_t r) {
  const uint32_t wi = r >> 5;
  uint32_t lo = a0, hi = a1;
  lo = (wi == 1u) ? a1 : lo;
  hi = (wi == 1u) ? a2 : hi;
  lo = (wi == 2u) ? a2 : lo;
  hi = (wi == 2u) ? a3 : hi;
  lo = (wi == 3u) ? a3 : lo;
  hi = (wi == 3u) ? a4 : hi;
  return __builtin_amdgcn_alignbit(hi, lo, r & 31u);
}

#define F8_MAXSEG 1800u
#define F8_LIST 32u

__device__ __forceinline__ static bool seg_table_f8(ParSmem& S, const BitSrc& src, uint32_t limit, uint32_t base, uint32_t stop,
                                                    const Lit8& f8, SegTab& tab, unsigned long long* dp) {
#define T8STAMP(i)                                                                  \
  do {                                                                              \
// ... 591 lines not shown
        const uint32_t adv = 8u * nlit;
        ob += nlit;
        b.bb >>= adv;
        b.nb -= adv;
        b.pos += adv;
      }
    }
    if (act && b.pos >= stop) act = false;
    lb_refill<LDS>(b, src);
    const uint32_t e = lut_l_entry(S, (uint32_t)b.bb);
    const uint32_t kind = (e >> 8) & 3u;
    const uint32_t cl = e & 15u, xb = (e >> 4) & 15u;
    uint32_t adv = cl + xb;
    bool bad = (kind == 3u) || (cl == 0u);
    uint32_t len = (e >> 16) + (((uint32_t)(b.bb >> cl)) & ((1u << xb) - 1u));
    uint32_t dist = 0;
    const bool ismatch = act && kind == 2u;
    if (__ballot(ismatch)) {
      LaneBits t = b;
      t.bb >>= adv;
      t.nb -= adv;
      t.pos += adv;
      lb_refill<LDS>(t, src);
      const uint32_t ed = lut_d_entry(S, (uint32_t)t.bb);
      const uint32_t dl = ed & 15u, dx = (ed >> 4) & 15u;
      dist = (ed >> 16) + (((uint32_t)(t.bb >> dl)) & ((1u << dx) - 1u));
      bad = bad || (kind == 2u && ((((ed >> 8) & 3u) != 2u) || dl == 0u));
      if (ismatch) {
        b = t;
        adv = dl + dx;
      }
    }
    adv = act ? adv : 0u;
    b.bb >>= adv;
    b.nb -= adv;
    b.pos += adv;
    if (act && (bad || b.pos > limit)) {
      fl |= F_FAIL;
      act = false;
    }
    if (act && kind == 1u) {
      fl |= F_EOB;
      act = false;
    }
    if (act) {
      if (kind == 0u) {
        if (ACC) {
          put((e >> 16) & 255u, 1u);
        } else if (EMIT) {
          const uint32_t q = out_off + ob - clo;
          if (!HIST || q < PAR_CHUNK) S.out[q] = (uint8_t)(e >> 16);
        }
        ob += 1u;
      } else {
        if (ACC) flush();
        if (EMIT) {
          const uint32_t p = out_off + ob, q = p - clo;
          if (!HIST && dist > p) {
            fl |= F_HIST;
          } else if (!HIST || q < PAR_CHUNK) {
            S.out[q] = (uint8_t)(dist - 1u);
            S.out[q + 1] = (uint8_t)((dist - 1u) >> 8);
            S.out[q + 2] = (uint8_t)(len - 3u);
            atomicOr(&S.bitmap[q >> 5], 1u << (q & 31u));
          } else if (p < clo && p + len > clo) {
            S.res_strad[0] = p + len - clo;
            S.res_strad[1] = dist;
          }
        }
        ob += len;
      }
      if (ob > (HIST ? PAR_MAX_OUT : ZES_BLK)) {
        fl |= F_FAIL;
        act = false;
      }
    }
  }
  if (ACC) flush();
  exit_pos = b.pos;
  outbytes = ob;
  flags = fl;
}

__device__ __forceinline__ static bool par_build(ParSmem& S, uint32_t base, uint32_t nsym, uint32_t chunk, bool is_dist, uint16_t* syms, uint32_t* first,
                                                 uint16_t* cnt, uint16_t* offs) {
  const uint32_t lane = zes_lane();
  const uint8_t* lens = S.lens + base;
  uint32_t c[16], before[16];
#pragma unroll
  for (int l = 0; l < 16; l++) c[l] = before[l] = 0;
  uint32_t myl = 0;
  for (uint32_t s0 = 0; s0 < nsym; s0 += 64) {
    const uint32_t s = s0 + lane;
    const uint32_t l = s < nsym ? lens[s] : 0u;
    if (s0 == 64u * chunk) {
      myl = l;
#pragma unroll
      for (int k = 1; k < 16; k++) before[k] = c[k];
    }
#pragma unroll
    for (int k = 1; k < 16; k++) c[k] += (uint32_t)__popcll(__ballot(l == (uint32_t)k));
  }
  uint32_t code = 0, off = 0, kraft = 0;
  uint32_t fst[16], ofs[16];
#pragma unroll
  for (int l = 1; l < 16; l++) {
    fst[l] = code;
    ofs[l] = off;
    code = (code + c[l]) << 1;
    off += c[l];
    kraft += c[l] << (15 - l);
  }
  if (kraft > 32768u) return false;
  if (chunk == 0u) {
    if (!is_dist) {
      uint32_t n8 = 0;
      for (uint32_t s0 = 0; s0 < 256u; s0 += 64) n8 += (uint32_t)__popcll(__ballot(lens[s0 + lane] == 8u));
      if (lane == 0) {
        S.f8lo = fst[8];
        S.f8n = n8 >= 128u ? n8 : 0u;
        S.f8off = ofs[8];
      }
    }
    if (lane < 16) {
      uint32_t f = 0, o2 = 0, cc = 0;
#pragma unroll
      for (int l = 1; l < 16; l++)
        if ((int)lane == l) {
          f = fst[l];
          o2 = ofs[l];
          cc = c[l];
        }
      first[lane] = f;
      offs[lane] = (uint16_t)o2;
      cnt[lane] = (uint16_t)cc;
    }
  }
  uint64_t same = ~0ull;
#pragma unroll
  for (int bt = 0; bt < 4; bt++) {
    const bool bit = (myl >> bt) & 1u;
    const uint64_t bal = __ballot(bit);
    same &= bit ? bal : ~bal;
  }
  if (myl) {
    uint32_t o2 = 0;
#pragma unroll
    for (int k = 1; k < 16; k++)
      if ((int)myl == k) o2 = ofs[k] + before[k];
    syms[o2 + (uint32_t)__popcll(same & zes_lanemask_lt())] = (uint16_t)(64u * chunk + lane);
  }
  return true;
}
template <uint32_t ROOT, bool IS_DIST>
__device__ __forceinline__ static void par_fill(uint32_t i, const uint16_t* syms, const uint32_t* first, const uint16_t* cnt, const uint16_t* offs,
                                                uint32_t* lut, uint8_t* blut) {
  uint32_t fst[ROOT + 1], cn[ROOT + 1], ofs[ROOT + 1];
#pragma unroll
  for (uint32_t l = 1; l <= ROOT; l++) {
    fst[l] = first[l];
    cn[l] = cnt[l];
    ofs[l] = offs[l];
  }
  const uint32_t msb = __brev(i) >> (32u - ROOT);
  uint32_t at = 0, len = 0;
#pragma unroll
// ... 180 lines not shown
    if (bad && lane == 0) atomicOr(&S.status, 1u);
    if (!past && !bad) {
      uint64_t m = 0;
      uint32_t cur = en, nsym = 0;
      while (cur < 64u) {
        const uint32_t v = (uint32_t)__builtin_amdgcn_readlane((int)pk, (int)cur);
        m |= 1ull << cur;
        nsym++;
        cur = v & 127u;
      }
      asm volatile("s_waitcnt lgkmcnt(0)" ::: "memory");
      if ((m >> lane) & 1ull) s_cl[(uint32_t)__popcll(m & zes_lanemask_lt())] = pk;
      asm volatile("s_waitcnt lgkmcnt(0)" ::: "memory");
      const uint32_t tc = s_cl[lane];
      const bool on = lane < nsym;
      const uint32_t s1 = on ? (tc >> 15) & 31u : 0u, r1 = on ? (tc >> 7) & 255u : 0u;
      const bool hole = on && !((tc >> 20) & 1u);
      const uint32_t is16 = (uint32_t)(on && !hole && s1 == 16u);
      const uint32_t valraw = s1 >= 16u ? 0u : s1;
      const uint32_t srcl = ph_scan_max((on && !is16) ? lane + 1u : 0u);
      const uint32_t vsrc = (uint32_t)__builtin_amdgcn_ds_bpermute((int)((srcl ? srcl - 1u : 0u) << 2), (int)valraw);
      const uint32_t val = srcl ? vsrc : prev;
      const uint32_t kin = ph_scan_add(r1);
      const uint32_t kk = k + kin - r1;
      const uint64_t endm = __ballot(on && !hole && kk + r1 >= total);
      const uint32_t cut = endm ? (uint32_t)__builtin_ctzll(endm) : nsym - 1u;
      const bool mine = on && lane <= cut;
      const uint64_t badm = __ballot(mine && (hole || (is16 && kk == 0u) || kk + r1 > total));
      if (badm) {
        if (lane == 0) atomicOr(&S.status, 1u);
      } else {
        if (mine && val) {
          for (uint32_t q = 0; q < r1; q++) {
            const uint32_t idx = kk + q;
            S.lens[idx < HLIT ? idx : 288 + (idx - HLIT)] = (uint8_t)val;
          }
        }
        if (endm) {
          const uint32_t nx = (uint32_t)__builtin_amdgcn_readlane((int)(tc & 127u), (int)cut);
          if (lane == 0) {
            S.hdr_end = wb + nx;
            S.h_done = 1;
          }
        } else if (wave == PAR_WAVES - 1u && lane == 0) {
          S.h_off = cur - 64u;
          S.h_k = (uint32_t)__builtin_amdgcn_readlane((int)(kk + r1), (int)cut);
          S.h_prev = (uint32_t)__builtin_amdgcn_readlane((int)val, (int)cut);
        }
      }
    }
    __syncthreads();
    if (S.status || S.h_done) break;
    off0 = S.h_off;
    k0 = S.h_k;
    prev0 = S.h_prev;
    wbase0 += 64u * PAR_WAVES;
    __syncthreads();
  }
  if (wave == 0) HSTAMP(2);
  if (!S.status && S.hdr_end > limit && threadIdx.x == 0) S.status = 1;
}

struct ParItem {
  const uint32_t* g32;
  uint32_t lastdw, limit, start;
  uint32_t de_est, de_est2;
  ZesCandRes* cres;
  ZesCandRes* cres_host;
  uint32_t* start_host;
  uint8_t* dst;
  uint64_t room;
  ZesSegRes* sres;
  uint32_t* sym;
  uint64_t sym_cap;
  uint32_t* sym_all;
  unsigned long long* bump;
  uint64_t bump_base, bump_cap;
  uint64_t* symoff;
  uint32_t* map;
  const uint32_t* cand;
  uint32_t ncand;
  uint32_t* fail_list;
  uint32_t w;
};

template <bool FOREIGN, bool TWO>
__device__ __forceinline__ static void par_body(ParSmem& S, const ParItem& it, unsigned long long* dbg) {
#define STAMP(i)                                                     \
  do {                                                               \
    if (dbg && threadIdx.x == 0) dbg[(size_t)blockIdx.x * ZES_PAR_DBG_ROW + (i)] = (unsigned long long)clock64(); \
  } while (0)
#define PAR_DECLINE(END_BIT, TOTAL)                                   \
  do {                                                                \
    if (threadIdx.x == 0) {                                           \
      if (FOREIGN) {                                                  \
        ZesSegRes r_;                                                 \
        r_.end_bit = 0;                                               \
        r_.out_len = 0;                                               \
        r_.flags = 0;                                                 \
        r_.next = 0;                                                  \
        *it.sres = r_;                                                \
        it.fail_list[1u + atomicAdd(&it.fail_list[0], 1u)] = it.w;    \
      } else {                                                        \
        ZesCandRes r_;                                                \
        r_.end_bit = (END_BIT);                                       \
        r_.out_len = (TOTAL);                                         \
        r_.flags = 0;                                                 \
        *it.cres = r_;                                                \
        if (it.cres_host) {                                           \
          *it.cres_host = r_;                                         \
          *it.start_host = it.start;                                  \
        }                                                             \
      }                                                               \
    }                                                                 \
  } while (0)
  const uint32_t tid = threadIdx.x, lane = tid & 63u, wave = tid >> 6;
  const uint32_t lastdw = it.lastdw, limit = it.limit, start = it.start;
  BitSrc src;
  src.g32 = it.g32;
  src.lastdw = lastdw;
  src.s32 = reinterpret_cast<const uint32_t*>(S.out);
  src.s_first = start >> 5;
  uint32_t ds = 0, seg0 = 0, seglen = 0, base = 0, stop = 0, ecode = 0, tail_code = 0;
  uint32_t plimit = limit;
  Lit8 f8 = {0, 0, 0};
  bool p2_global = false;
  STAMP(0);
  auto stage_and_tables = [&](const uint32_t de_est) __attribute__((always_inline)) -> uint32_t {
    {
      const uint64_t end_bit = min((uint64_t)limit, max((uint64_t)de_est, (uint64_t)start + 4800u) + 1280u);
      const uint32_t end_dw = min(lastdw, (uint32_t)((end_bit + 63u) >> 5));
      src.s_count = end_dw - src.s_first + 1u;
      plimit = (uint32_t)min((uint64_t)limit, ((uint64_t)end_dw + 1u) * 32u);
    }
    const bool use_lds = src.s_count <= STAGE_DW;
    if (tid == 0) S.status = use_lds ? 0u : 1u;
    if (use_lds) {
      uint32_t* st = reinterpret_cast<uint32_t*>(S.out);
      for (uint32_t k = tid; k < src.s_count; k += PAR_THREADS) st[k ^ ((k >> 5) & 31u)] = src.g32[src.s_first + k];
    }
    __syncthreads();
    unsigned long long* hdbg = dbg ? dbg + (size_t)blockIdx.x * ZES_PAR_DBG_ROW : nullptr;
    if (wave == 0 && use_lds) {
      const bool ok = par_header_fixed<true>(S, src, plimit, start, hdbg);
      if (!ok && lane == 0) S.status = 1;
    }
    __syncthreads();
    if (S.status) return 1u;
    par_header_lens<true>(S, src, plimit, hdbg);
    __syncthreads();
    if (S.status) return 1u;
    if (wave < 5u) {
      if (!par_build(S, 0, 288, wave, false, S.syms_l, S.first_l, S.cnt_l, S.offs_l) && lane == 0) atomicOr(&S.status, 1u);
    } else if (wave == 5u) {
      if (!par_build(S, 288, 32, 0, true, S.syms_d, S.first_d, S.cnt_d, S.offs_d) && lane == 0) atomicOr(&S.status, 1u);
    }
    __syncthreads();
    if (wave == 0) HSTAMP(3);
    if (S.status) return 1u;
    static_assert(PAR_THREADS == (1u << PL_ROOT) && PAR_THREADS >= (1u << PD_ROOT), "one thread per root-table entry");
    par_fill<PL_ROOT, false>(tid, S.syms_l, S.first_l, S.cnt_l, S.offs_l, S.lut_l, S.len_l);
    if (tid < (1u << PD_ROOT)) par_fill<PD_ROOT, true>(tid, S.syms_d, S.first_d, S.cnt_d, S.offs_d, S.lut_d, S.len_d);
    __syncthreads();
    if (wave == 0) HSTAMP(4);
    STAMP(1);
    ds = S.hdr_end;
    if (!FOREIGN && TWO) {
      if (wave == 0) {
        LaneBits pb;
        lb_seek<true>(pb, src, ds + lane);
        uint32_t v = 0, len = 0, dist = 0;
        const uint32_t kind = (ds + lane < plimit) ? tok_step<true>(S, pb, src, v, len, dist) : T_FAIL;
        const uint32_t w0 = kind | ((pb.pos - (ds + lane)) << 2) | (len << 8);
        uint32_t cur = 0, made = 0;
        bool hist = false;
        for (uint32_t k = 0; k < 16u && cur < 64u; k++) {
          const uint32_t a = (uint32_t)__builtin_amdgcn_readlane((int)w0, (int)cur);
          const uint32_t d = (uint32_t)__builtin_amdgcn_readlane((int)dist, (int)cur);
          const uint32_t kd = a & 3u;
          if (kd == T_LIT) {
            made++;
          } else if (kd == T_MATCH) {
            if (d > made) {
              hist = true;
              break;
            }
            made += (a >> 8) & 511u;
          } else {
            break;
          }
          cur += (a >> 2) & 63u;
        }
        if (hist && lane == 0) S.status = 1u;
      }
      __syncthreads();
      if (S.status) return 1u;
    }
    f8.lo = S.f8lo;
    f8.n = S.f8n;
    f8.off = S.f8off;
    const uint32_t tab_off = ((src.s_count + 31u) & ~31u) * 4u;
    {
      const uint32_t span = de_est > ds ? de_est - ds : 1u;
      seglen = max(64u, (span + PAR_THREADS - 1) / PAR_THREADS);
    }
    const bool dp = TWO && tab_off + DP_BYTES <= STAGE_DW * 4u && !(f8.n && seglen >= 256u);
    seg0 = ds;
    if (dp) {
      seg0 = ds & ~31u;
      const uint32_t span = de_est > seg0 ? de_est - seg0 : 1u;
      seglen = (max(64u, (span + PAR_THREADS - 1) / PAR_THREADS) + 31u) & ~31u;
    }

    const uint64_t b_me64 = (uint64_t)seg0 + (uint64_t)tid * seglen;
    base = (uint32_t)(b_me64 < 0xFFFFFF00ull ? b_me64 : 0xFFFFFF00ull);
    stop = (uint32_t)((b_me64 + seglen) < 0xFFFFFF00ull ? (b_me64 + seglen) : 0xFFFFFF00ull);
    SegTab tab = {0, 0, 0, 0, 0, 0, 0, 0};
    if (dp) {
      uint8_t* T13 = S.out + tab_off + PAR_THREADS * DP_ROW;
      uint8_t* D12 = T13 + (1u << DP_LROOT);
      dp_build(S, T13, D12);
      __syncthreads();
      seg_table_dp(S, src, plimit, base, seglen, T13, D12, S.out + tab_off + tid * DP_ROW);
    } else {
      seg_table<true, TWO>(S, src, plimit, base, stop, f8, tab, dbg ? dbg + (size_t)blockIdx.x * ZES_PAR_DBG_ROW : nullptr);
    }
    STAMP(2);
    const bool room = dp || tab_off + PAR_THREADS * 52u <= STAGE_DW * 4u;
    const bool over = !room && !FOREIGN;
    const bool lds_tabs = room || over;
    const uint32_t toff = over ? 0u : tab_off;
    p2_global = over;
    const uint32_t tstride = dp ? DP_ROW : 52u;
    const uint8_t* tb = S.out + toff + wave * 64u * tstride;
    if (over) __syncthreads();
    if (dp) {
      __syncthreads();
    } else if (lds_tabs) {
      uint32_t* tw = reinterpret_cast<uint32_t*>(S.out + toff) + tid * 13u;
      tw[0] = (uint32_t)tab.a;
      tw[1] = (uint32_t)(tab.a >> 32);
      tw[2] = (uint32_t)tab.b;
      tw[3] = (uint32_t)(tab.b >> 32);
      tw[4] = (uint32_t)tab.c;
      tw[5] = (uint32_t)(tab.c >> 32);
      tw[6] = (uint32_t)tab.d;
      tw[7] = (uint32_t)(tab.d >> 32);
      tw[8] = (uint32_t)tab.e;
      tw[9] = (uint32_t)(tab.e >> 32);
      tw[10] = (uint32_t)tab.f;
      tw[11] = (uint32_t)(tab.f >> 32);
      __syncthreads();
    }
    {
      uint32_t cur = lane;
      if (lds_tabs) {
        uint8_t* gt = &S.gtab[wave][0][0];
#pragma unroll
        for (uint32_t q = 0; q < 3u; q++) {
          const uint32_t idx = lane + 64u * q, grp = idx / 48u, j = idx - 48u * grp;
          uint32_t c = j;
          for (uint32_t sgm = 0; sgm < 16u; sgm++) {
            const uint32_t v = tb[(16u * grp + sgm) * tstride + (c < 48u ? c : 0u)];
            c = c < 48u ? v : c;
          }
          gt[idx] = (uint8_t)c;
        }
        asm volatile("s_waitcnt lgkmcnt(0)" ::: "memory");
#pragma unroll
        for (uint32_t grp = 0; grp < 4u; grp++) {
          const uint32_t v = gt[48u * grp + (cur < 48u ? cur : 0u)];
          cur = cur < 48u ? v : cur;
        }
      } else {
        for (uint32_t sgm = 0; sgm < 64u; sgm++) {
          const SegTab ws = tab_bcast(tab, sgm);
          if (cur < 48u) cur = tab_get(ws, cur);
        }
      }
      if (lane < 48u) S.wtab[wave][lane] = (uint8_t)cur;
    }
    __syncthreads();
    if (tid == 0) {
      uint32_t e = ds - seg0;
      for (uint32_t k = 0; k < PAR_WAVES; k++) {
        S.wentry[k] = (uint8_t)e;
        if (e < 48u) e = S.wtab[k][e];
      }
      S.tail_entry = e;
    }
    __syncthreads();
    uint32_t e = (uint32_t)__builtin_amdgcn_readfirstlane((int)S.wentry[wave]);
    uint32_t mine = C_FAIL;
    if (lds_tabs) {
      const uint8_t* gt = &S.gtab[wave][0][0];
      const uint32_t grp = lane >> 4, upto = lane & 15u;
      uint32_t eg = e, c = e;
#pragma unroll
      for (uint32_t k = 0; k < 3u; k++) {
        eg = eg < 48u ? (uint32_t)gt[48u * k + eg] : eg;
        c = grp == k + 1u ? eg : c;
      }
      for (uint32_t sgm = 0; sgm < 15u; sgm++) {
        const uint32_t v = tb[(16u * grp + sgm) * tstride + (c < 48u ? c : 0u)];
        c = (sgm < upto && c < 48u) ? v : c;
      }
      mine = c;
    } else {
      for (uint32_t sgm = 0; sgm < 64u; sgm++) {
        if (lane == sgm) mine = e;
        const uint32_t own = e < 48u ? tab_get(tab, e) : e;
        e = (uint32_t)__builtin_amdgcn_readlane((int)own, (int)sgm);
      }
    }
    ecode = mine;
    tail_code = S.tail_entry;
    return 0u;
  };
  uint32_t bad = stage_and_tables(it.de_est);
  if (!bad && (tail_code < 48u || tail_code == C_FAIL) && it.de_est2) {
    __syncthreads();
    bad = stage_and_tables(it.de_est2);
  }
  if (bad) {
    PAR_DECLINE(start, 0u);
    return;
  }
  STAMP(3);

  uint32_t entry = base + ecode, exit_pos = 0, outbytes = 0, flags = 0;
  if (!FOREIGN && p2_global)
    seg_run<false, false, FOREIGN>(S, src, plimit, entry, stop, ecode < 48u, f8, 0, exit_pos, outbytes, flags);
  else
    seg_run<false, true, FOREIGN>(S, src, plimit, entry, stop, ecode < 48u, f8, 0, exit_pos, outbytes, flags);
  STAMP(22);
  if (dbg && threadIdx.x == PAR_THREADS - 64) dbg[(size_t)blockIdx.x * ZES_PAR_DBG_ROW + 23] = (unsigned long long)clock64();
  if (ecode >= 48u) flags = F_VOID;
  if (tid == 0) {
    S.tail_bytes = 0;
    S.tail_end = 0;
  }
  __syncthreads();
  for (uint32_t i = tid; i < ZES_BLK / 32; i += PAR_THREADS) S.bitmap[i] = 0;
  uint32_t tail_start = 0;
  if (tail_code < 48u) {
    const uint64_t last_stop = (uint64_t)seg0 + (uint64_t)PAR_THREADS * seglen;
    tail_start = (uint32_t)(last_stop + tail_code);
    if (tid == 0) {
      uint32_t ex, ob, fl;
      seg_decode<false, false, FOREIGN>(S, src, limit, tail_start, 0xFFFFFF00u, 0, ex, ob, fl);
      S.tail_bytes = ob;
      S.tail_end = ex;
      if (!(fl & F_EOB) || (fl & F_FAIL)) atomicOr(&S.status, 2u);
      else atomicOr(&S.status, 4u);
    }
  } else if (tail_code == C_FAIL) {
    if (tid == 0) atomicOr(&S.status, 2u);
  }
  {
    uint32_t incl = outbytes;
#pragma unroll
    for (int dlt = 1; dlt < 64; dlt <<= 1) {
      const uint32_t t = __shfl_up(incl, dlt);
      if ((int)lane >= dlt) incl += t;
    }
    if (lane == 63) S.wave_sum[wave] = incl;
    const uint64_t eobm = __ballot((flags & F_EOB) && !(flags & F_VOID));
    const uint64_t failm = __ballot((flags & F_FAIL) && !(flags & F_VOID));
    if (failm && lane == 0) atomicOr(&S.status, 2u);
    if (eobm && lane == (uint32_t)__builtin_ctzll(eobm)) {
      atomicOr(&S.status, 4u);
      S.hdr_end = exit_pos;
    }
    __syncthreads();
    uint32_t wbase = 0, total = 0;
#pragma unroll
    for (uint32_t k = 0; k < PAR_WAVES; k++) {
      const uint32_t sm = S.wave_sum[k];
      if (k < wave) wbase += sm;
      total += sm;
    }
    const uint32_t seg_total = total;
    total += S.tail_bytes;
    const uint32_t st = S.status;
    const uint32_t end_bit = (tail_code < 48u) ? S.tail_end : S.hdr_end;
    const bool good = (st & 4u) && !(st & 2u) && total <= (FOREIGN ? PAR_MAX_OUT : ZES_BLK) && (FOREIGN || S.bfinal || total == ZES_BLK);
    if (!good) {
      PAR_DECLINE(end_bit, total);
      return;
    }
    const uint32_t my_off = wbase + incl - outbytes;
    STAMP(4);
    uint32_t* symp = it.sym;
    if (FOREIGN) {
      if ((uint64_t)total > it.sym_cap) {
        if (tid == 0) {
          const unsigned long long o = atomicAdd(it.bump, (unsigned long long)((total + 7u) & ~7u));
          S.sp_n = (o + total <= it.bump_cap) ? (uint32_t)(o >> 3) : 0xFFFFFFFFu;
        }
        __syncthreads();
        const uint32_t o8 = S.sp_n;
        __syncthreads();
        if (o8 == 0xFFFFFFFFu) {
          PAR_DECLINE(end_bit, total);
          return;
        }
        symp = it.sym_all + it.bump_base + (uint64_t)o8 * 4u;
      }
      if (tid == 0) *it.symoff = (uint64_t)(symp - it.sym_all);
    }

    uint32_t clo = 0;
    static_assert(PAR_CHUNK % RES_W == 0 && PAR_DIST_OFF + 2u * RES_W <= ZES_BLK, "T2: the distance array lies behind the chunk");
  next_chunk:
    const uint32_t clen = FOREIGN ? min(PAR_CHUNK, total - clo) : total;
    if (FOREIGN) {
      if (tid < 4u) S.res_strad[tid] = 0u;
      if (clo) {
        for (uint32_t i = tid; i < ZES_BLK / 32; i += PAR_THREADS) S.bitmap[i] = 0;
      }
      __syncthreads();
    }
    uint32_t f2 = 0;
    {
      uint32_t ex2, ob2;
      const Lit8 f8e = (FOREIGN && total > PAR_CHUNK) ? Lit8{0, 0, 0} : f8;
      const bool inchunk = !FOREIGN || (my_off < clo + PAR_CHUNK && my_off + outbytes > clo);
      seg_run<true, false, FOREIGN>(S, src, limit, entry, stop, !(flags & F_VOID) && entry < stop && inchunk, f8e, my_off, ex2, ob2, f2, clo);
    }
    if (tid == 0 && tail_code < 48u) {
      uint32_t ex2, ob2, f3 = 0;
      seg_decode<true, false, FOREIGN>(S, src, limit, tail_start, 0xFFFFFF00u, seg_total, ex2, ob2, f3, clo);
      f2 |= f3;
    }
    if (f2 & F_HIST) atomicOr(&S.status, 8u);
    __syncthreads();
    if (S.status & 8u) {
      PAR_DECLINE(end_bit, total);
      return;
    }

    STAMP(5);
    {
      uint16_t* dist = FOREIGN ? reinterpret_cast<uint16_t*>(S.out + PAR_DIST_OFF) : reinterpret_cast<uint16_t*>(S.lut_l);
      if (tid < 3u) S.res_flag[tid] = 0u;
      if (!FOREIGN && tid < 4u) S.res_strad[tid] = 0u;
      __syncthreads();
      unsigned long long tacc[4] = {0, 0, 0, 0}, tlast = dbg ? clock64() : 0ull, nrounds = 0;
#define P4LAP(i)                                         \
  do {                                                   \
    if (dbg && tid == 0) {                               \
      const unsigned long long now_ = clock64();         \
      tacc[i] += now_ - tlast;                           \
      tlast = now_;                                      \
    }                                                    \
  } while (0)
      bool sparse_done = false;
      uint32_t nstarts = 0;
      if (!FOREIGN) {
        static_assert(sizeof(S.lut_l) >= P4_SPARSE_MAX * 4u && sizeof(S.lut_d) >= P4_SPARSE_MAX, "the lists lie over the dead decode tables");
        uint32_t* sp_list = S.lut_l;
        uint8_t* sp_dep = reinterpret_cast<uint8_t*>(S.lut_d);
        uint32_t bw[ZES_BLK / 32 / PAR_THREADS], cnt4 = 0;
#pragma unroll
        for (uint32_t k = 0; k < ZES_BLK / 32 / PAR_THREADS; k++) {
          bw[k] = S.bitmap[tid * (ZES_BLK / 32 / PAR_THREADS) + k];
          cnt4 += (uint32_t)__popc(bw[k]);
        }
        uint32_t incl = cnt4;
#pragma unroll
        for (int dlt = 1; dlt < 64; dlt <<= 1) {
          const uint32_t t = __shfl_up(incl, dlt);
          if ((int)lane >= dlt) incl += t;
        }
        __syncthreads();
        if (lane == 63) S.wave_sum[wave] = incl;
        __syncthreads();
        uint32_t wbase2 = 0, nm = 0;
#pragma unroll
        for (uint32_t k = 0; k < PAR_WAVES; k++) {
          const uint32_t sm = S.wave_sum[k];
          if (k < wave) wbase2 += sm;
          nm += sm;
        }
        nstarts = nm;
        auto rec_of = [&](uint32_t P, uint32_t& D, uint32_t& L) {
          D = ((uint32_t)S.out[P] | ((uint32_t)S.out[P + 1u] << 8)) + 1u;
          L = (uint32_t)S.out[P + 2u] + 3u;
        };
        if (tid == 0) S.sp_n = 0;
        if (nm <= P4_SPARSE_MAX) {
          uint32_t kk = wbase2 + incl - cnt4;
#pragma unroll
          for (uint32_t k = 0; k < ZES_BLK / 32 / PAR_THREADS; k++) {
            uint32_t w = bw[k];
            while (w) {
              const uint32_t bit = (uint32_t)__builtin_ctz(w);
              w &= w - 1u;
              sp_list[kk++] = 32u * (tid * (ZES_BLK / 32 / PAR_THREADS) + k) + bit;
            }
          }
          __syncthreads();
          if (tid < nm) {
            uint32_t P = sp_list[tid], D, L;
            rec_of(P, D, L);
            const uint32_t a = P - D, b = a + min(D, L);
            const uint32_t from = a > (ZES_MAXMATCH - 1u) ? a - (ZES_MAXMATCH - 1u) : 0u;
            uint32_t lo = 0, hi = nm;
            while (lo < hi) {
              const uint32_t mid = (lo + hi) >> 1;
              if (sp_list[mid] < from) lo = mid + 1u; else hi = mid;
// ... 326 lines not shown
        }
        it.map[i2] = v[0] | (v[1] << 16);
      }
      if (tid == 0) {
        ZesSegRes r;
        r.end_bit = end_bit;
        r.out_len = total;
        r.flags = 1u | (fin ? 2u : 0u);
        r.next = next;
        *it.sres = r;
      }
    }
    STAMP(7);
  }
}

#undef PAR_DECLINE
#undef STAMP

template <bool TWO>
__device__ __forceinline__ static void block_par_t1(ParSmem& S, const uint8_t* __restrict__ d_in, uint8_t* __restrict__ d_out,
                                                    const ZesInfBuf* __restrict__ bufs, uint32_t nbuf, const uint32_t* __restrict__ cnt,
                                                    const uint32_t* __restrict__ cand_all, const uint32_t* __restrict__ map_all,
                                                    ZesCandRes* __restrict__ cres_all, unsigned long long* __restrict__ dbg,
                                                    const uint32_t* __restrict__ redo, const uint32_t* __restrict__ raw_all,
                                                    uint32_t* __restrict__ sorted_all, const ZesParMirror& mir) {
  if (mir.counters_host && blockIdx.x == 0)
    for (uint32_t i = threadIdx.x; i < mir.counter_words; i += PAR_THREADS) mir.counters_host[i] = mir.counters[i];
  uint32_t bi = 0;
  {
    uint32_t lo = 0, hi = nbuf;
    while (hi - lo > 1) {
      const uint32_t mid = (lo + hi) >> 1;
      if (bufs[mid].work_first <= blockIdx.x) lo = mid; else hi = mid;
    }
    bi = lo;
  }
  uint32_t w = redo ? redo[blockIdx.x] : blockIdx.x - bufs[bi].work_first;
  const uint32_t ncand = min(cnt[bi], bufs[bi].cand_cap);
  uint32_t nwork = bufs[bi + 1].work_first - bufs[bi].work_first;
  if (bufs[nbuf].work_first == ZES_WORK_AUTO) {
    nwork = min(ncand, bufs[nbuf].cand_cap);
    if (blockIdx.x >= nwork) return;
  }
  const uint32_t* cand = cand_all + bufs[bi].cand_base;
  const uint32_t* map = map_all ? map_all + bufs[bi].cand_base : nullptr;
  uint32_t w_rank = 0, raw_next = 0xFFFFFFFFu, raw_next2 = 0xFFFFFFFFu, raw_min = 0, raw_mine = 0;
  const bool ranked = raw_all && !map_all && !redo;
  if (ranked) {
    const uint32_t* raw = raw_all + bufs[bi].cand_base;
    const uint32_t x = blockIdx.x - bufs[bi].work_first;
    if (x >= ncand) return;
    const uint32_t u = raw[x];
    if (threadIdx.x == 0) {
      S.wave_sum[0] = 0;
      S.wave_sum[1] = 0xFFFFFFFFu;
      S.wave_sum[2] = 0xFFFFFFFFu;
      S.wave_sum[3] = 0xFFFFFFFFu;
    }
    __syncthreads();
    uint32_t less = 0, nx = 0xFFFFFFFFu, mn = 0xFFFFFFFFu;
    for (uint32_t j = threadIdx.x; j < ncand; j += PAR_THREADS) {
      const uint32_t v = raw[j];
      less += (v < u || (v == u && j < x)) ? 1u : 0u;
      nx = (v > u && v < nx) ? v : nx;
      mn = min(mn, v);
    }
    if (less) atomicAdd(&S.wave_sum[0], less);
    if (nx != 0xFFFFFFFFu) atomicMin(&S.wave_sum[1], nx);
    atomicMin(&S.wave_sum[3], mn);
    __syncthreads();
    raw_next = S.wave_sum[1];
    uint32_t nx2 = 0xFFFFFFFFu;
    for (uint32_t j = threadIdx.x; j < ncand; j += PAR_THREADS) {
      const uint32_t v = raw[j];
      nx2 = (v > raw_next && v < nx2) ? v : nx2;
    }
    if (raw_next != 0xFFFFFFFFu && nx2 != 0xFFFFFFFFu) atomicMin(&S.wave_sum[2], nx2);
    __syncthreads();
    w_rank = S.wave_sum[0];
    raw_next2 = S.wave_sum[2];
    raw_min = S.wave_sum[3];
    raw_mine = u;
    if (threadIdx.x == 0) {
      sorted_all[bufs[bi].cand_base + w_rank] = u;
      if (mir.cres_host) {
        ZesCandRes r0;
        r0.end_bit = 0;
        r0.out_len = 0;
        r0.flags = 0;
        mir.cres_host[w_rank] = r0;
        mir.start_host[w_rank] = u + 16u;
      }
    }
    __syncthreads();
  }
  if (!map_all && !redo && (((ranked ? raw_min : cand[0]) != bufs[bi].start_rel && !(bufs[bi].range_flags & ZES_START_ANY)) || cnt[bi] > bufs[bi].cand_cap)) return;
  const uint64_t c = bufs[bi].c;
  if (ranked) w = w_rank;
  const uint32_t ci = map ? map[w] : w;
  if ((bufs[bi].range_flags & ZES_OWN_ONLY) && (ranked ? raw_mine : cand[ci]) >= bufs[bi].own_rel) return;
  ParItem it;
  it.g32 = reinterpret_cast<const uint32_t*>(d_in + bufs[bi].in_off);
  it.lastdw = (uint32_t)((c - 1) >> 2);
  it.limit = (uint32_t)(c * 8);
  it.start = (ranked ? raw_mine : cand[ci]) + 16u;
  it.de_est = it.limit;
  it.de_est2 = 0;
  if (ranked) {
    if (raw_next != 0xFFFFFFFFu) {
      it.de_est = raw_next + 16u;
      it.de_est2 = raw_next2 != 0xFFFFFFFFu ? raw_next2 + 16u : it.limit;
    }
  } else if (map) {
    if (w + 1 < nwork) it.de_est = cand[map[w + 1]] + 16u;
  } else if (ci + 1u < ncand) {
    it.de_est = cand[ci + 1u] + 16u;
    it.de_est2 = ci + 2u < ncand ? cand[ci + 2u] + 16u : it.limit;
  }
  it.cres = cres_all + bufs[bi].cand_base + w;
  it.cres_host = mir.cres_host ? mir.cres_host + w : nullptr;
  it.start_host = mir.cres_host ? mir.start_host + w : nullptr;
  const uint64_t slot_off = (uint64_t)w * ZES_BLK;
  it.dst = d_out + bufs[bi].out_off + slot_off;
  it.room = bufs[bi].cap > slot_off ? bufs[bi].cap - slot_off : 0;
  it.sres = nullptr;
  it.sym = nullptr;
  it.sym_cap = 0;
  it.sym_all = nullptr;
  it.bump = nullptr;
  it.bump_base = it.bump_cap = 0;
  it.symoff = nullptr;
  it.map = nullptr;
  it.cand = nullptr;
  it.ncand = 0;
  it.fail_list = nullptr;
  it.w = w;
  par_body<false, TWO>(S, it, dbg);
}

__global__ __launch_bounds__(PAR_THREADS) void k_inf_block_par(const uint8_t* __restrict__ d_in, uint8_t* __restrict__ d_out,
                                                               const ZesInfBuf* __restrict__ bufs, uint32_t nbuf,
                                                               const uint32_t* __restrict__ cnt, const uint32_t* __restrict__ cand_all,
                                                               const uint32_t* __restrict__ map_all, ZesCandRes* __restrict__ cres_all,
                                                               unsigned long long* __restrict__ dbg, const uint32_t* __restrict__ redo,
                                                               const uint32_t* __restrict__ raw_all, uint32_t* __restrict__ sorted_all, ZesParMirror mir) {
  __shared__ __align__(16) ParSmem S;
  block_par_t1<false>(S, d_in, d_out, bufs, nbuf, cnt, cand_all, map_all, cres_all, dbg, redo, raw_all, sorted_all, mir);
}
__global__ __launch_bounds__(PAR_THREADS) void k_inf_block_par2(const uint8_t* __restrict__ d_in, uint8_t* __restrict__ d_out,
                                                                const ZesInfBuf* __restrict__ bufs, uint32_t nbuf,
                                                                const uint32_t* __restrict__ cnt, const uint32_t* __restrict__ cand_all,
                                                                const uint32_t* __restrict__ map_all, ZesCandRes* __restrict__ cres_all,
                                                                unsigned long long* __restrict__ dbg, const uint32_t* __restrict__ redo,
                                                                const uint32_t* __restrict__ raw_all, uint32_t* __restrict__ sorted_all, ZesParMirror mir) {
  __shared__ __align__(16) ParSmem S;
  block_par_t1<true>(S, d_in, d_out, bufs, nbuf, cnt, cand_all, map_all, cres_all, dbg, redo, raw_all, sorted_all, mir);
}

__global__ __launch_bounds__(PAR_THREADS) void k_inf_seg_block_par(const uint8_t* __restrict__ d_in, const ZesSegJob* __restrict__ jobs,
                                                                   uint32_t njobs, const uint32_t* __restrict__ cand_all,
                                                                   ZesSegRes* __restrict__ sres_all, uint32_t* __restrict__ maps_all,
                                                                   uint32_t* __restrict__ sym16_all, uint32_t sym_ratio,
                                                                   uint32_t* __restrict__ fail_list, unsigned long long* __restrict__ bump,
                                                                   uint64_t bump_base, uint64_t bump_cap, uint64_t* __restrict__ symoff,
                                                                   unsigned long long* __restrict__ dbg) {
  __shared__ __align__(16) ParSmem S;
  uint32_t bi = 0;
  {
    uint32_t lo = 0, hi = njobs;
    while (hi - lo > 1) {
      const uint32_t mid = (lo + hi) >> 1;
      if (jobs[mid].work_first <= blockIdx.x) lo = mid; else hi = mid;
    }
    bi = lo;
  }
  const ZesSegJob jb = jobs[bi];
  const uint32_t w = blockIdx.x - jb.work_first;
  const uint32_t ncand = jb.ncand;
  const uint32_t* cand = cand_all + jb.cand_base;
  ZesSegRes* sres = sres_all + jb.work_first;
  const uint64_t c = jb.c;
  uint64_t start = jb.start0;
  if (w > 0) {
    const uint32_t c0 = cand[w - 1];
    if (c0 + 16u == jb.start0) {
      if (threadIdx.x == 0) {
        ZesSegRes r;
        r.end_bit = 0;
        r.out_len = 0;
        r.flags = 0;
        r.next = 0;
        sres[w] = r;
      }
      return;
    }
    start = (uint64_t)c0 + 16;
  }
  uint32_t nx = w;
  if (w == 0 && ncand > 0 && cand[0] + 16u == jb.start0) nx = 1;
  ParItem it;
  it.g32 = reinterpret_cast<const uint32_t*>(d_in + jb.in_off);
  it.lastdw = (uint32_t)((c - 1) >> 2);
  it.limit = (uint32_t)(c * 8);
  it.start = (uint32_t)start;
  it.de_est = nx < ncand ? cand[nx] + 16u : it.limit;
  it.de_est2 = nx < ncand ? (nx + 1u < ncand ? cand[nx + 1u] + 16u : it.limit) : 0u;
  it.cres = nullptr;
  it.cres_host = nullptr;
  it.start_host = nullptr;
  it.dst = nullptr;
  it.room = 0;
  it.sres = sres + w;
  const uint64_t b0 = (start - 16) / 8, b1 = nx < ncand ? (uint64_t)cand[nx] / 8 : c;
  it.sym = sym16_all + jb.sym_base + b0 * sym_ratio / 2;
  it.sym_cap = (b1 - b0) * sym_ratio;
  it.sym_all = sym16_all;
  it.bump = bump;
  it.bump_base = bump_base;
  it.bump_cap = bump_cap;
  it.symoff = symoff + blockIdx.x;
  it.map = maps_all + (size_t)jb.work_first * (ZES_WINDOW / 2) + (size_t)w * (ZES_WINDOW / 2);
  it.cand = cand;
  it.ncand = ncand;
  it.fail_list = fail_list;
  it.w = blockIdx.x;
  par_body<true, true>(S, it, dbg);
}
```

zlib.es_amd/csrc/zes_kernels.h:

```cpp
#pragma once
#include "zes_common.h"

#define SORT_THREADS 1024
#define SORT_WAVES (SORT_THREADS / 64)
#ifndef MATCH_THREADS
#define MATCH_THREADS 1024
#endif
#define IDX_THREADS 1024
#define ZES_SORT_LAZY 0x80000000u
#define ZES_SORT_INDEX 0x40000000u
#define ZES_SORT_REDO 0x20000000u
#define ZES_INV_NONE 0xFFFFFFFFu
#define ZES_ROUTE_WORDS 9u
#define ZES_ROUTE_SORT_TWO 1u
#define ZES_ROUTE_SORT_DENSE 2u
#define ZES_ROUTE_IDX_MAXC 0x3FFFFu
#define ZES_ROUTE_IDX_GROUP 0x40000000u
#define ZES_ROUTE_IDX_HEAVY 0x80000000u
#define ZES_ROUTE_GUARDED 1u
#define ZES_ROUTE_PROBED 2u
#define ZES_ROUTE_PERIODIC 4u
#define ZES_ROUTE_ABORT3 8u
#define ZES_ROUTE_LATE_CLEAR 16u
#define ZES_ROUTE_WALK3 32u
#define PARSE_THREADS 1024
#define EMIT_THREADS 1024
#define HUFF_THREADS_HOST 256
#define ADLER_THREADS 256
#define ADLER_CHUNK 65536u
#define CRC_THREADS 256u
#define CRC_PIECES 16u
#define CRC_CHUNK (CRC_THREADS * CRC_PIECES * 16u)
#define CRC_STRIDE (CRC_THREADS * 16u)
#define CRC_TAB_FOLD 512u
#define CRC_TAB_LANE 640u
#define CRC_TAB_POW (CRC_TAB_LANE + CRC_THREADS)
#define ZES_PAR_DBG_ROW 32
#define ZES_TMASK_WORDS (131072 / 32 + 4)
#define ZES_MLIST_CAP 4095u
#define ZES_MLIST_WORDS 4096u
#define PAR_THREADS 1024
#define PAR_WAVES (PAR_THREADS / 64)
#define INF_SCAN_THREADS 256
#ifndef INF_SCAN_BYTES
#define INF_SCAN_BYTES 8192u
#endif
#define SEG_BUCKETS 2048u

struct ZesInfBuf {
  uint64_t in_off, c, out_off, cap;
  uint32_t first_chunk;
  uint32_t cand_base;
  uint32_t cand_cap;
  uint32_t work_first;
  uint32_t start_rel;
  uint32_t own_rel;
  uint32_t range_flags;
  uint32_t pad;
};
#define ZES_START_ANY 1u
#define ZES_OWN_ONLY 2u

#define ZES_WORK_AUTO 0xFFFFFFFFu

struct ZesCandRes {
  uint64_t end_bit;
  uint32_t out_len;
  uint32_t flags;
};

struct ZesParMirror {
  ZesCandRes* cres_host;
  uint32_t* start_host;
  const uint32_t* counters;
  uint32_t* counters_host;
  uint32_t counter_words;
};

struct ZesSegRes {
  uint64_t end_bit;
  uint64_t out_len;
  uint32_t flags;
  uint32_t next;
};

struct ZesStoredBlk {
  uint64_t src, dst;
  uint32_t len, pad;
};

struct ZesSegJob {
  uint64_t in_off, c;
  uint64_t sym_base;
  uint32_t cand_base;
  uint32_t ncand;
  uint32_t work_first;
  uint32_t nseg;
  uint32_t start0;
  uint32_t flags;
};
#define ZES_SEG_PARTIAL 1u

struct ZesSegOut {
  uint64_t out_off, cap;
  uint32_t nseg;
  uint32_t hist;
};

struct ZesCrcSeg {
  uint64_t off, len;
};

struct ZesGzMember {
  uint32_t size;
  uint32_t hlen;
  uint32_t crc;
  uint32_t isize;
};
struct ZesGzWalk {
  uint32_t count;
  uint32_t ok;
  uint64_t end;
};
#define ZES_GZ_HLEN_MAX 256u
#define ZES_BGZF_MARK_TILE 16384u
#define ZES_BGZF_MARK_THREADS 256u
struct ZesBgzfCand {
  uint64_t pos;
  uint32_t size;
  uint32_t hlen;
  uint32_t crc;
  uint32_t isize;
};
struct ZesBgzfMark {
  uint32_t count;
  uint32_t pad[3];
};
struct ZesGzSeg {
  uint64_t src_off, dst_off, len;
  uint32_t zhdr;
  uint32_t pad;
};
#define GZ_GATHER_THREADS 256u
#define GZ_GATHER_PIECE 65536u
struct ZesBgzfRec {
  uint64_t src_off;
  uint64_t dst_off;
  uint32_t body_len;
  uint32_t len;
  uint32_t crc;
  uint32_t kind;
};
#define ZES_BGZF_STREAM 0u
#define ZES_BGZF_STORED 1u
#define ZES_BGZF_EOF 2u
#define ZES_BGZF_HLEN 18u
struct ZesZipRec {
  uint64_t hdr_at;
  uint64_t name_at;
  uint64_t limit;
  uint64_t dst_off;
  uint32_t csize;
  uint16_t name_len, method;
  uint32_t flag0;
  uint32_t pad;
};
struct ZesZipVerdict {
  int32_t status;
  uint32_t pad;
  uint64_t data_off;
};
struct ZesZipPackRec {
  uint64_t src_off;
  uint64_t dst_off;
  uint32_t csize;
  uint32_t usize;
  uint32_t crc;
  uint32_t name_off;
  uint32_t first_wg;
  uint16_t name_len, method, flags, pad;
  uint32_t pad2;
};
#define ZES_ZIP_PACK_SHARES 1024u

uint32_t zes_crc_shift(uint32_t s, uint64_t k);
uint32_t zes_crc_mul(uint32_t a, uint32_t b);
uint32_t zes_crc_host(const uint8_t* p, uint64_t n);
void zes_crc_tables(uint32_t* tab, uint32_t npow);

#ifdef __HIPCC__
__global__ void k_inf_first_bytes(const uint8_t*, const uint64_t*, uint8_t*, uint32_t);
__global__ void k_inf_scan(const uint8_t*, const ZesInfBuf*, uint32_t, unsigned long long*, uint32_t, uint32_t*, uint8_t*, uint32_t,
                           const uint8_t*);
__global__ void k_inf_set_table1(ZesInfBuf, ZesInfBuf, ZesInfBuf*, uint32_t*, uint32_t);
__global__ void k_inf_verify(const uint8_t*, const ZesInfBuf*, const unsigned long long*, uint32_t, uint32_t*, uint32_t*, uint32_t*, uint32_t, uint32_t*, uint32_t, uint32_t);
__global__ void k_inf_verify_long(const uint8_t*, const ZesInfBuf*, const unsigned long long*, uint32_t, uint32_t*, uint32_t*, uint32_t*, uint32_t, const uint32_t*, uint32_t);
__global__ void k_inf_ranksort(const ZesInfBuf*, const uint32_t*, const uint32_t*, uint32_t*, uint32_t);
__global__ void k_inf_decode(const uint8_t*, uint8_t*, const ZesInfBuf*, ZesRes*, uint64_t*);
__global__ void k_inf_stored_walk(const uint8_t*, uint64_t, uint64_t, uint64_t, ZesStoredBlk*, ZesRes*);
__global__ void k_inf_stored_copy(const uint8_t*, uint64_t, uint8_t*, uint64_t, const ZesStoredBlk*);
__global__ void k_inf_stored_find(const uint8_t*, uint64_t, uint32_t, uint32_t*, uint32_t*);
__global__ void k_inf_stored_rank(const uint8_t*, uint64_t, uint32_t, const uint32_t*, const uint32_t*, uint32_t, uint64_t, ZesStoredBlk*, ZesRes*);
__global__ void k_inf_cand_bucket(const uint32_t*, const uint32_t*, uint32_t, uint32_t, uint32_t*);
__global__ void k_inf_cand_compact(const uint32_t*, uint32_t*, uint32_t*);
__global__ void k_inf_seg_order(const ZesSegJob*, const uint32_t*, uint32_t*);
__global__ void k_inf_seg_scan(const uint8_t*, const ZesSegJob*, uint32_t, const uint32_t*, ZesSegRes*, uint32_t*, uint32_t*, uint32_t,
                               const uint32_t*, uint32_t*, const uint32_t*, uint64_t*);
__global__ void k_inf_seg_scan_short(const uint8_t*, const ZesSegJob*, uint32_t, const uint32_t*, ZesSegRes*, uint32_t*, uint32_t*, uint32_t,
                                     const uint32_t*, uint32_t*, const uint32_t*, uint64_t*);
__global__ void k_inf_seg_block_par(const uint8_t*, const ZesSegJob*, uint32_t, const uint32_t*, ZesSegRes*, uint32_t*, uint32_t*, uint32_t, uint32_t*,
                                    unsigned long long*, uint64_t, uint64_t, uint64_t*, unsigned long long*);
__global__ void k_inf_seg_chain(const ZesSegJob*, const ZesSegRes*, uint32_t*, uint64_t*, ZesRes*, uint32_t*);
__global__ void k_inf_seg_translate(uint8_t*, const ZesSegJob*, const ZesSegOut*, const uint32_t*, const ZesSegRes*, const uint32_t*, const uint64_t*,
                                    const uint8_t*, const uint32_t*, const uint64_t*, uint32_t*);
#define SEGWIN_GROUP 32u
__global__ void k_inf_seg_win_group(const uint32_t*, const uint32_t*, const ZesSegJob*, uint32_t*);
__global__ void k_inf_seg_win_top(const uint32_t*, const ZesSegJob*, uint8_t*, const uint8_t*, const ZesSegOut*);
__global__ void k_inf_seg_win_fin(const uint32_t*, const ZesSegJob*, const uint8_t*, uint8_t*);
__global__ void k_inf_seg_decode(const uint8_t*, uint64_t, uint64_t, uint8_t*, uint64_t, uint64_t, const uint32_t*, const ZesSegRes*,
                                 const uint32_t*, const uint64_t*, const uint8_t*, uint32_t*, uint32_t, uint32_t, uint32_t);
__global__ void k_inf_block_par(const uint8_t*, uint8_t*, const ZesInfBuf*, uint32_t, const uint32_t*, const uint32_t*, const uint32_t*,
                                ZesCandRes*, unsigned long long*, const uint32_t*, const uint32_t*, uint32_t*, ZesParMirror);
__global__ void k_inf_block_par2(const uint8_t*, uint8_t*, const ZesInfBuf*, uint32_t, const uint32_t*, const uint32_t*, const uint32_t*,
                                ZesCandRes*, unsigned long long*, const uint32_t*, const uint32_t*, uint32_t*, ZesParMirror);
__global__ void k_inf_move_slots(uint8_t*, const uint8_t*, const uint32_t*, const uint32_t*, uint32_t);
__global__ void k_inf_chain(const ZesInfBuf*, const uint32_t*, const uint32_t*, const ZesCandRes*, const uint32_t*, uint32_t*, ZesRes*, const uint32_t*, uint32_t, uint32_t*);
__global__ void k_inf_chain_range(const ZesInfBuf*, const uint32_t*, const uint32_t*, const ZesCandRes*, ZesRes*, unsigned long long*);
__global__ void k_inf_set_table_range(ZesInfBuf, ZesInfBuf, ZesInfBuf*, uint32_t*, uint32_t, const unsigned long long*, unsigned long long);
__global__ void k_inf_exact(const uint8_t*, uint64_t, uint64_t, uint8_t*, uint64_t, uint64_t, const uint64_t*, ZesRes*);
void zes_sort_set_dbg(unsigned long long*);
#ifdef WD_PROFILE
void zes_wd_set_dbg(unsigned long long*);
#endif
void zes_parse_set_dbg(unsigned long long*);
void zes_lazy_set_dbg(unsigned long long*);
void zes_huff_set_dbg(unsigned long long*);
__global__ void k_make_blks(ZesBuf, uint32_t, ZesBuf*, ZesBlk*, uint32_t, unsigned long long*);
__global__ void k_lz_sort(const uint8_t*, const ZesBuf*, const ZesBlk*, uint32_t*, uint32_t*, uint32_t*, uint16_t*, uint32_t);
__global__ void k_lz_index(const uint8_t*, const ZesBuf*, const ZesBlk*, uint32_t*, uint32_t*, uint32_t*, uint16_t*);
#define ZES_SORT_MODE_FIRST 0u
#define ZES_SORT_MODE_REDO 1u
#define ZES_SORT_USE_INDEX 256u
__global__ void k_lz_match_lazy(const uint8_t*, const ZesBuf*, const ZesBlk*, const uint32_t*, const uint32_t*, const uint16_t*, uint32_t*, uint32_t*, uint32_t*,
                                const uint32_t*);
__global__ void k_lz_order(const uint32_t*, uint32_t, uint32_t*);
__global__ void k_lz_match(const uint8_t*, const ZesBuf*, const ZesBlk*, const uint32_t*, uint32_t*, uint32_t*);
__global__ void k_lz_parse(const uint8_t*, const ZesBuf*, ZesBlk*, const uint32_t*, uint32_t*, uint32_t*, const uint32_t*, const uint32_t*);
__global__ void k_lz_parse_small(const uint8_t*, const ZesBuf*, ZesBlk*, const uint32_t*, uint32_t*, uint32_t*, const uint32_t*, const uint32_t*);
__global__ void k_huff(ZesBlk*, const uint32_t*, uint32_t*, uint32_t*);
__global__ void k_huff_lengths_only(const uint32_t*, uint32_t, uint32_t, uint8_t*);
__global__ void k_selftest_lds_order(unsigned long long*, uint32_t, uint32_t);
__global__ void k_adler(const uint8_t*, uint64_t, uint64_t, unsigned long long*);
__global__ void k_crc32(const uint8_t*, uint64_t, const uint32_t*, unsigned int*);
__global__ void k_crc32_seg(const uint8_t*, const ZesCrcSeg*, const uint2*, const uint32_t*, unsigned int*);
__global__ void k_gz_walk(const uint8_t*, uint64_t, ZesGzWalk*, ZesGzMember*, uint32_t);
__global__ void k_bgzf_mark(const uint8_t*, uint64_t, ZesBgzfMark*, ZesBgzfCand*, uint32_t);
__global__ void k_gz_gather(const uint8_t*, uint8_t*, const ZesGzSeg*);
__global__ void k_bgzf_pack(const uint8_t*, const uint8_t*, uint8_t*, const ZesBgzfRec*);
__global__ void k_zip_stage(const uint8_t*, uint8_t*, uint8_t*, const ZesZipRec*, ZesZipVerdict*);
__global__ void k_zip_pack(const uint8_t*, const uint8_t*, const uint8_t*, uint8_t*, const ZesZipPackRec*, uint32_t);
__global__ void k_adler_blocks(const uint8_t*, const ZesBuf*, const ZesBlk*, unsigned long long*);
__global__ void k_adler_seg(const uint8_t*, const ZesCrcSeg*, const uint2*, unsigned long long*);
__global__ void k_layout(uint8_t*, const ZesBuf*, ZesBlk*, const unsigned long long*, ZesRes*);
__global__ void k_emit(uint8_t*, const ZesBuf*, const ZesBlk*, const uint32_t*, const uint32_t*, const uint32_t*);
__global__ void k_zero_u64(unsigned long long*, uint32_t);
__global__ void k_bits_place(uint32_t*, uint64_t, const uint32_t*, uint64_t);
#endif
```

Measured before the change: 45.61 GiB/s.

## Decode parallel-inflate segments from a register-resident bit window

Adds seg_run_win, a segment decoder that loads each lane's compressed segment (up to 36 dwords) into registers once and extracts bits with alignbit. This replaces repeated source loads in both the scan pass and the emit pass of the block-parallel inflate. It also marks several block-uniform values with readfirstlane so they can live in scalar registers. The costs are much higher VGPR pressure, which may lower occupancy, and an extra device counter and debug API that tally how often the window path is taken. The path can be disabled with ZES_PAR_REGBITS=0.

```diff
diff --git a/include/zes.h b/include/zes.h
--- a/include/zes.h
+++ b/include/zes.h
@@ -157,6 +157,7 @@
 typedef struct zes_ktime { const char* name; float ms; uint32_t launches; } zes_ktime;
 int zes_last_kernel_times(zes_ktime* out, int cap);
 int zes_last_inflate_tier(void);
+uint32_t zes_debug_last_par_regbits(void);
 int zes_last_gunzip_members(void);
 int zes_set_profiling(int on);
 
diff --git a/zlib.es_amd/__init__.py b/zlib.es_amd/__init__.py
--- a/zlib.es_amd/__init__.py
+++ b/zlib.es_amd/__init__.py
@@ -93,6 +93,8 @@
             getattr(L, name).argtypes = [C.c_void_p, C.c_uint64, u32p]
         L.zes_crc32_batch_dev.argtypes = [C.c_void_p, u64p, u64p, u32p, C.c_uint32]
         L.zes_last_gunzip_members.argtypes = []
+        L.zes_debug_last_par_regbits.restype = C.c_uint32
+        L.zes_debug_last_par_regbits.argtypes = []
         L.zes_gzip_bound.argtypes = [C.c_uint64, u64p]
         for name in ("zes_gzip", "zes_gzip_dev"):
             getattr(L, name).argtypes = [C.c_void_p, C.c_uint64, C.c_void_p, C.c_uint64, u64p]
@@ -841,6 +843,10 @@
     return int(lib().zes_last_inflate_tier())
 
 
+def last_par_regbits():
+    return int(lib().zes_debug_last_par_regbits())
+
+
 def last_gunzip_members():
     return int(lib().zes_last_gunzip_members())
 
diff --git a/zlib.es_amd/csrc/zes_api.hip b/zlib.es_amd/csrc/zes_api.hip
--- a/zlib.es_amd/csrc/zes_api.hip
+++ b/zlib.es_amd/csrc/zes_api.hip
@@ -177,6 +177,7 @@
 #undef X
   uint32_t crc_npow = 0;
   DevBuf kraft;
+  DevBuf regbits;
   PinnedArea* pinned = nullptr;
   PinnedArea* pinned_dev = nullptr;
   ParMirror* mirror = nullptr;
@@ -304,6 +305,9 @@
     g.kraft.cap = 4096;
     HIPCHK(hipMemcpy(g.kraft.p, tab, 4096, hipMemcpyHostToDevice));
   }
+  HIPCHK(hipMalloc(&g.regbits.p, 64));
+  g.regbits.cap = 64;
+  HIPCHK(hipMemset(g.regbits.p, 0, 64));
   g.device = device;
   g.ready = true;
   return ZES_OK;
@@ -1116,7 +1120,7 @@
   t.cnt = t.counters + 4;
   if (t.one) {
     hipLaunchKernelGGL(k_inf_set_table1, dim3(1), dim3(64), 0, g.stream, hb[0], hb[1], (ZesInfBuf*)g.ibufs.p, t.counters,
-                       (uint32_t)(t.cnt_bytes / 4));
+                       (uint32_t)(t.cnt_bytes / 4), (uint32_t*)g.regbits.p);
   } else {
     HIPCHK(hipMemcpyAsync(g.ibufs.p, hb, sizeof(ZesInfBuf) * (nbuf + 1), hipMemcpyHostToDevice, g.stream));
     HIPCHK(hipMemsetAsync(g.counters.p, 0, t.cnt_bytes, g.stream));
@@ -1165,6 +1169,12 @@
     mir.counter_words = (uint32_t)(t.cnt_bytes / 4);
     t.hostchain = true;
   }
+  static const bool no_regbits = [] {
+    const char* e = getenv("ZES_PAR_REGBITS");
+    return e && e[0] == '0' && e[1] == 0;
+  }();
+  if (no_regbits) mir.flags |= ZES_PAR_NO_REGBITS;
+  if (t.one) mir.regbits_n = (uint32_t*)g.regbits.p;
   launch_block_par(two ? "k_inf_block_par2" : "k_inf_block_par", two, (uint32_t)t.work, t.d_in, t.d_out, t.dbufs, nbuf, t.cnt, t.dbg, nullptr, mir);
   return ZES_OK;
 }
@@ -1971,7 +1981,7 @@
   ZesInfBuf b1;
   memset(&b1, 0, sizeof b1);
   b1.first_chunk = chunks;
-  hipLaunchKernelGGL(k_inf_set_table1, dim3(1), dim3(64), 0, g.stream, b0, b1, const_cast<ZesInfBuf*>(G.dbufs), G.counters, 4u);
+  hipLaunchKernelGGL(k_inf_set_table1, dim3(1), dim3(64), 0, g.stream, b0, b1, const_cast<ZesInfBuf*>(G.dbufs), G.counters, 4u, (uint32_t*)nullptr);
   const bool reuse = G.nb == 1 && g.sv.holds(g.surv, G.d_in, b0.in_off, b0.c) && b0.start_rel == 0u && g.sv.n <= G.surv_cap;
   g.sv.drop();
   if (reuse) {
@@ -2157,7 +2167,7 @@
     {
       const ZesInfBuf b0 = inf_buf(j);
       if ((rc = ensure(g.ibufs, sizeof(ZesInfBuf) * 2))) return rc;
-      hipLaunchKernelGGL(k_inf_set_table1, dim3(1), dim3(64), 0, g.stream, b0, b0, (ZesInfBuf*)g.ibufs.p, (uint32_t*)nullptr, 0u);
+      hipLaunchKernelGGL(k_inf_set_table1, dim3(1), dim3(64), 0, g.stream, b0, b0, (ZesInfBuf*)g.ibufs.p, (uint32_t*)nullptr, 0u, (uint32_t*)nullptr);
       Timed t("k_inf_decode_seq");
       hipLaunchKernelGGL(k_inf_decode, dim3(1), dim3(64), 0, g.stream, d_in, d_out, (const ZesInfBuf*)g.ibufs.p, (ZesRes*)g.res.p,
                          (uint64_t*)g.resume.p);
@@ -2610,6 +2620,7 @@
   (void)hipStreamSynchronize(g.stream);
   free_scratch_locked();
   (void)release(g.kraft);
+  (void)release(g.regbits);
   if (g.pinned) (void)hipHostFree(g.pinned);
   if (g.mirror) (void)hipHostFree(g.mirror);
   if (g.res_more) (void)hipHostFree(g.res_more);
@@ -5094,6 +5105,16 @@
   return g.last_tier;
 }
 
+uint32_t zes_debug_last_par_regbits(void) {
+  UseDev ud(t_last);
+  std::lock_guard<std::mutex> lk(g_mu);
+  if (!g.ready) return 0;
+  (void)hipSetDevice(g.device);
+  uint32_t n = 0;
+  if (hipStreamSynchronize(g.stream) != hipSuccess || hipMemcpy(&n, g.regbits.p, 4, hipMemcpyDeviceToHost) != hipSuccess) return 0xFFFFFFFFu;
+  return n;
+}
+
 int zes_last_gunzip_members(void) {
   UseDev ud(t_last);
   std::lock_guard<std::mutex> lk(g_mu);
diff --git a/zlib.es_amd/csrc/zes_inflate.hip b/zlib.es_amd/csrc/zes_inflate.hip
--- a/zlib.es_amd/csrc/zes_inflate.hip
+++ b/zlib.es_amd/csrc/zes_inflate.hip
@@ -33,10 +33,11 @@
 }
 
 __global__ void k_inf_set_table1(ZesInfBuf b0, ZesInfBuf sentinel, ZesInfBuf* __restrict__ bufs, uint32_t* __restrict__ counters,
-                                 uint32_t nwords) {
+                                 uint32_t nwords, uint32_t* __restrict__ word) {
   if (threadIdx.x == 0) {
     bufs[0] = b0;
     bufs[1] = sentinel;
+    if (word) *word = 0;
   }
   if (counters && threadIdx.x < nwords) counters[threadIdx.x] = 0;
 }
diff --git a/zlib.es_amd/csrc/zes_inflate_par.hip b/zlib.es_amd/csrc/zes_inflate_par.hip
--- a/zlib.es_amd/csrc/zes_inflate_par.hip
+++ b/zlib.es_amd/csrc/zes_inflate_par.hip
@@ -193,16 +193,19 @@
   return r;
 }
 
+template <bool ONE_BASE = false>
 __device__ __forceinline__ static int slow_sym(const LaneBits& b, uint32_t root, const uint16_t* syms, const uint32_t* first,
                                                const uint16_t* cnt, const uint16_t* offs, uint32_t* len_out) {
   uint32_t code = __brev((uint32_t)b.bb & ((1u << root) - 1u)) >> (32u - root);
+  uint32_t z = 0;
+  if (ONE_BASE) asm volatile("" : "+v"(z));
   for (uint32_t len = root + 1; len <= 15u; len++) {
     code = (code << 1) | (uint32_t)((b.bb >> (len - 1)) & 1u);
-    const uint32_t f = first[len];
+    const uint32_t f = first[len + z];
     const uint32_t rel = code - f;
-    if (code >= f && rel < cnt[len]) {
+    if (code >= f && rel < cnt[len + z]) {
       *len_out = len;
-      return (int)syms[offs[len] + rel];
+      return (int)syms[offs[len + z] + rel];
     }
   }
   return -1;
@@ -252,24 +255,26 @@
   return T_MATCH;
 }
 
+template <bool ONE_BASE = false>
 __device__ __forceinline__ static uint32_t lut_l_entry(ParSmem& S, uint32_t bits) {
   uint32_t e = S.lut_l[bits & ((1u << PL_ROOT) - 1u)];
   if ((e & 15u) == 0u) {
     LaneBits t;
     t.bb = bits;
     uint32_t l2 = 0;
-    const int sy = slow_sym(t, PL_ROOT, S.syms_l, S.first_l, S.cnt_l, S.offs_l, &l2);
+    const int sy = slow_sym<ONE_BASE>(t, PL_ROOT, S.syms_l, S.first_l, S.cnt_l, S.offs_l, &l2);
     e = sy < 0 ? 0u : entry_l((uint32_t)sy, l2);
   }
   return e;
 }
+template <bool ONE_BASE = false>
 __device__ __forceinline__ static uint32_t lut_d_entry(ParSmem& S, uint32_t bits) {
   uint32_t e = S.lut_d[bits & ((1u << PD_ROOT) - 1u)];
   if ((e & 15u) == 0u) {
     LaneBits t;
     t.bb = bits;
     uint32_t l2 = 0;
-    const int sy = slow_sym(t, PD_ROOT, S.syms_d, S.first_d, S.cnt_d, S.offs_d, &l2);
+    const int sy = slow_sym<ONE_BASE>(t, PD_ROOT, S.syms_d, S.first_d, S.cnt_d, S.offs_d, &l2);
     e = sy < 0 ? 0u : entry_d((uint32_t)sy, l2);
   }
   return e;
@@ -1027,6 +1032,131 @@
   flags = fl;
 }
 
+#define SEG_DW 36u
+#define SEG_WIN_MAXLEN (32u * SEG_DW - 48u - 31u)
+#ifndef SEG_TURN
+#define SEG_TURN 2u
+#endif
+static_assert(SEG_TURN == 1u || SEG_TURN == 2u, "a turn's dword is picked by one bit of the lane's position");
+static_assert(SEG_DW % SEG_TURN == 0u, "whole turns");
+
+template <bool EMIT>
+__device__ __forceinline__ static void seg_run_win(ParSmem& S, const uint32_t (&r)[SEG_DW], uint32_t d0, uint32_t limit, uint32_t entry,
+                                                   uint32_t stop, bool live, const Lit8& f8, uint32_t out_off, uint32_t& exit_pos,
+                                                   uint32_t& outbytes, uint32_t& flags) {
+  uint32_t pos = live ? entry : 0u;
+  const uint32_t wbit = 32u * d0;
+  uint32_t ob = 0, fl = 0;
+  bool act = live && pos < stop;
+  uint32_t pend = 0, pn = 0;
+  auto put = [&](uint32_t v, uint32_t n) __attribute__((always_inline)) {
+    uint32_t P = out_off + ob;
+    v &= n >= 4u ? ~0u : ((1u << (8u * n)) - 1u);
+    if (pn == 0u && (P & 3u) != 0u && n != 0u) {
+      const uint32_t k = min(n, 4u - (P & 3u));
+      for (uint32_t i = 0; i < k; i++) S.out[P + i] = (uint8_t)(v >> (8u * i));
+      v = k < 4u ? v >> (8u * k) : 0u;
+      n -= k;
+      P += k;
+    }
+    const uint64_t w = (uint64_t)pend | ((uint64_t)v << (8u * pn));
+    const uint32_t t = pn + n;
+    if (t >= 4u) *reinterpret_cast<uint32_t*>(S.out + (P - pn)) = (uint32_t)w;
+    pend = t >= 4u ? (uint32_t)(w >> 32) : (uint32_t)w;
+    pn = t >= 4u ? t - 4u : t;
+  };
+  auto flush = [&]() __attribute__((always_inline)) {
+    const uint32_t P = out_off + ob - pn;
+    for (uint32_t i = 0; i < pn; i++) S.out[P + i] = (uint8_t)(pend >> (8u * i));
+    pend = 0;
+    pn = 0;
+  };
+#define SEG_R(i) ((i) < SEG_DW ? r[(i) < SEG_DW ? (i) : 0u] : 0u)
+#pragma unroll
+  for (uint32_t t = 0; t < SEG_DW / SEG_TURN; t++) {
+    const uint32_t j = SEG_TURN * t, tend = 32u * SEG_TURN * (t + 1u);
+    while (__ballot(act && pos < wbit + tend)) {
+      const bool in = act && pos < wbit + tend;
+      const bool up = SEG_TURN == 2u && ((pos ^ wbit) & 32u) != 0u;
+      const uint32_t w0 = up ? SEG_R(j + 1u) : SEG_R(j), w1 = up ? SEG_R(j + 2u) : SEG_R(j + 1u), w2 = up ? SEG_R(j + 3u) : SEG_R(j + 2u);
+      const uint32_t lo = __builtin_amdgcn_alignbit(w1, w0, pos & 31u), hi = __builtin_amdgcn_alignbit(w2, w1, pos & 31u);
+      const bool fast = in && pos + 32u <= stop && pos + 32u <= limit && ob + 4u <= ZES_BLK;
+      const uint32_t nlit = fast ? lead_lit8(lo, f8) : 0u;
+      if (EMIT && nlit) {
+        const uint32_t rv = __brev(lo);
+        const uint32_t k0 = f8.off - f8.lo;
+        const uint32_t i0 = k0 + (rv >> 24), i1 = k0 + ((rv >> 16) & 255u), i2 = k0 + ((rv >> 8) & 255u), i3 = k0 + (rv & 255u);
+        const uint32_t s0 = S.syms_l[i0], s1 = S.syms_l[nlit > 1u ? i1 : i0], s2 = S.syms_l[nlit > 2u ? i2 : i0],
+                       s3 = S.syms_l[nlit > 3u ? i3 : i0];
+        put((s0 & 255u) | ((s1 & 255u) << 8) | ((s2 & 255u) << 16) | (s3 << 24), nlit);
+      }
+      ob += nlit;
+      pos += 8u * nlit;
+      bool gen = in && nlit == 0u;
+      if (__ballot(gen)) {
+        const uint64_t bb = (uint64_t)lo | ((uint64_t)hi << 32);
+        const uint32_t e = lut_l_entry<true>(S, lo);
+        const uint32_t kind = (e >> 8) & 3u;
+        const uint32_t cl = e & 15u, xb = (e >> 4) & 15u;
+        uint32_t adv = cl + xb;
+        bool bad = (kind == 3u) || (cl == 0u);
+        const uint32_t len = (e >> 16) + (((uint32_t)(bb >> cl)) & ((1u << xb) - 1u));
+        uint32_t dist = 0;
+        const bool ismatch = gen && kind == 2u;
+        if (__ballot(ismatch)) {
+          const uint64_t tb = bb >> adv;
+          const uint32_t ed = lut_d_entry<true>(S, (uint32_t)tb);
+          const uint32_t dl = ed & 15u, dx = (ed >> 4) & 15u;
+          dist = (ed >> 16) + (((uint32_t)(tb >> dl)) & ((1u << dx) - 1u));
+          bad = bad || (kind == 2u && ((((ed >> 8) & 3u) != 2u) || dl == 0u));
+          adv += ismatch ? dl + dx : 0u;
+        }
+        adv = gen ? adv : 0u;
+        pos += adv;
+        if (gen && (bad || pos > limit)) {
+          fl |= F_FAIL;
+          act = gen = false;
+        }
+        if (gen && kind == 1u) {
+          fl |= F_EOB;
+          act = gen = false;
+        }
+        if (gen) {
+          if (kind == 0u) {
+            if (EMIT) put((e >> 16) & 255u, 1u);
+            ob += 1u;
+          } else {
+            if (EMIT) {
+              flush();
+              const uint32_t p = out_off + ob;
+              if (dist > p) {
+                fl |= F_HIST;
+              } else {
+                S.out[p] = (uint8_t)(dist - 1u);
+                S.out[p + 1] = (uint8_t)((dist - 1u) >> 8);
+                S.out[p + 2] = (uint8_t)(len - 3u);
+                atomicOr(&S.bitmap[p >> 5], 1u << (p & 31u));
+              }
+            }
+            ob += len;
+          }
+          if (ob > ZES_BLK) {
+            fl |= F_FAIL;
+            act = false;
+          }
+        }
+      }
+      if (act && pos >= stop) act = false;
+    }
+    if (!__ballot(act)) break;
+  }
+#undef SEG_R
+  if (EMIT) flush();
+  exit_pos = pos;
+  outbytes = ob;
+  flags = fl;
+}
+
 __device__ __forceinline__ static bool par_build(ParSmem& S, uint32_t base, uint32_t nsym, uint32_t chunk, bool is_dist, uint16_t* syms, uint32_t* first,
                                                  uint16_t* cnt, uint16_t* offs) {
   const uint32_t lane = zes_lane();
@@ -1373,7 +1503,11 @@
   uint32_t ncand;
   uint32_t* fail_list;
   uint32_t w;
+  bool regbits;
+  uint32_t* regbits_n;
 };
+
+__device__ __forceinline__ static uint32_t par_uniform(uint32_t v) { return (uint32_t)__builtin_amdgcn_readfirstlane((int)v); }
 
 template <bool FOREIGN, bool TWO>
 __device__ __forceinline__ static void par_body(ParSmem& S, const ParItem& it, unsigned long long* dbg) {
@@ -1416,6 +1550,13 @@
   uint32_t plimit = limit;
   Lit8 f8 = {0, 0, 0};
   bool p2_global = false;
+  constexpr bool WIN = !FOREIGN && !TWO;
+  uint32_t win[SEG_DW];
+  bool p23_win = false;
+  auto win_drop = [&]() __attribute__((always_inline)) {
+#pragma unroll
+    for (uint32_t i = 0; i < SEG_DW; i++) win[i] = 0u;
+  };
   STAMP(0);
   auto stage_and_tables = [&](const uint32_t de_est) __attribute__((always_inline)) -> uint32_t {
     {
@@ -1490,6 +1631,11 @@
     f8.lo = S.f8lo;
     f8.n = S.f8n;
     f8.off = S.f8off;
+    if (WIN) {
+      f8.lo = par_uniform(f8.lo);
+      f8.n = par_uniform(f8.n);
+      f8.off = par_uniform(f8.off);
+    }
     const uint32_t tab_off = ((src.s_count + 31u) & ~31u) * 4u;
     {
       const uint32_t span = de_est > ds ? de_est - ds : 1u;
@@ -1524,6 +1670,18 @@
     p2_global = over;
     const uint32_t tstride = dp ? DP_ROW : 52u;
     const uint8_t* tb = S.out + toff + wave * 64u * tstride;
+    if (WIN) {
+      const bool fits = it.regbits && over && f8.n != 0u && seglen <= SEG_WIN_MAXLEN && (uint64_t)seg0 + (uint64_t)PAR_THREADS * seglen < 0xFFFFFF00ull;
+      p23_win = __builtin_amdgcn_readfirstlane((int)fits) != 0;
+      if (p23_win) {
+#pragma unroll
+        for (uint32_t i = 0; i < SEG_DW; i++) {
+          win[i] = src_ldw<true>(src, (base >> 5) + i);
+        }
+      } else {
+        win_drop();
+      }
+    }
     if (over) __syncthreads();
     if (dp) {
       __syncthreads();
@@ -1605,7 +1763,7 @@
       }
     }
     ecode = mine;
-    tail_code = S.tail_entry;
+    tail_code = WIN ? par_uniform(S.tail_entry) : S.tail_entry;
     return 0u;
   };
   uint32_t bad = stage_and_tables(it.de_est);
@@ -1620,10 +1778,16 @@
   STAMP(3);
 
   uint32_t entry = base + ecode, exit_pos = 0, outbytes = 0, flags = 0;
-  if (!FOREIGN && p2_global)
-    seg_run<false, false, FOREIGN>(S, src, plimit, entry, stop, ecode < 48u, f8, 0, exit_pos, outbytes, flags);
-  else
-    seg_run<false, true, FOREIGN>(S, src, plimit, entry, stop, ecode < 48u, f8, 0, exit_pos, outbytes, flags);
+  if (WIN && p23_win) {
+    if (tid == 0 && it.regbits_n) atomicAdd(it.regbits_n, 1u);
+    seg_run_win<false>(S, win, base >> 5, plimit, entry, stop, ecode < 48u, f8, 0, exit_pos, outbytes, flags);
+  } else {
+    if (!FOREIGN && p2_global)
+      seg_run<false, false, FOREIGN>(S, src, plimit, entry, stop, ecode < 48u, f8, 0, exit_pos, outbytes, flags);
+    else
+      seg_run<false, true, FOREIGN>(S, src, plimit, entry, stop, ecode < 48u, f8, 0, exit_pos, outbytes, flags);
+    if (WIN) win_drop();
+  }
   STAMP(22);
   if (dbg && threadIdx.x == PAR_THREADS - 64) dbg[(size_t)blockIdx.x * ZES_PAR_DBG_ROW + 23] = (unsigned long long)clock64();
   if (ecode >= 48u) flags = F_VOID;
@@ -1671,10 +1835,11 @@
       if (k < wave) wbase += sm;
       total += sm;
     }
-    const uint32_t seg_total = total;
-    total += S.tail_bytes;
+    const uint32_t seg_total = WIN ? par_uniform(total) : total;
+    total = WIN ? par_uniform(seg_total + S.tail_bytes) : seg_total + S.tail_bytes;
     const uint32_t st = S.status;
-    const uint32_t end_bit = (tail_code < 48u) ? S.tail_end : S.hdr_end;
+    const uint32_t end_bit_v = (tail_code < 48u) ? S.tail_end : S.hdr_end;
+    const uint32_t end_bit = WIN ? par_uniform(end_bit_v) : end_bit_v;
     const bool good = (st & 4u) && !(st & 2u) && total <= (FOREIGN ? PAR_MAX_OUT : ZES_BLK) && (FOREIGN || S.bfinal || total == ZES_BLK);
     if (!good) {
       PAR_DECLINE(end_bit, total);
@@ -1717,7 +1882,10 @@
       uint32_t ex2, ob2;
       const Lit8 f8e = (FOREIGN && total > PAR_CHUNK) ? Lit8{0, 0, 0} : f8;
       const bool inchunk = !FOREIGN || (my_off < clo + PAR_CHUNK && my_off + outbytes > clo);
-      seg_run<true, false, FOREIGN>(S, src, limit, entry, stop, !(flags & F_VOID) && entry < stop && inchunk, f8e, my_off, ex2, ob2, f2, clo);
+      if (WIN && p23_win)
+        seg_run_win<true>(S, win, base >> 5, limit, entry, stop, !(flags & F_VOID) && entry < stop, f8, my_off, ex2, ob2, f2);
+      else
+        seg_run<true, false, FOREIGN>(S, src, limit, entry, stop, !(flags & F_VOID) && entry < stop && inchunk, f8e, my_off, ex2, ob2, f2, clo);
     }
     if (tid == 0 && tail_code < 48u) {
       uint32_t ex2, ob2, f3 = 0;
@@ -2210,6 +2378,13 @@
     raw_next2 = S.wave_sum[2];
     raw_min = S.wave_sum[3];
     raw_mine = u;
+    if (!TWO) {
+      w_rank = par_uniform(w_rank);
+      raw_next = par_uniform(raw_next);
+      raw_next2 = par_uniform(raw_next2);
+      raw_min = par_uniform(raw_min);
+      raw_mine = par_uniform(raw_mine);
+    }
     if (threadIdx.x == 0) {
       sorted_all[bufs[bi].cand_base + w_rank] = u;
       if (mir.cres_host) {
@@ -2264,6 +2439,8 @@
   it.ncand = 0;
   it.fail_list = nullptr;
   it.w = w;
+  it.regbits = !(mir.flags & ZES_PAR_NO_REGBITS);
+  it.regbits_n = mir.regbits_n;
   par_body<false, TWO>(S, it, dbg);
 }
 
@@ -2353,5 +2530,7 @@
   it.ncand = ncand;
   it.fail_list = fail_list;
   it.w = blockIdx.x;
+  it.regbits = false;
+  it.regbits_n = nullptr;
   par_body<true, true>(S, it, dbg);
 }
diff --git a/zlib.es_amd/csrc/zes_kernels.h b/zlib.es_amd/csrc/zes_kernels.h
--- a/zlib.es_amd/csrc/zes_kernels.h
+++ b/zlib.es_amd/csrc/zes_kernels.h
@@ -75,7 +75,10 @@
   const uint32_t* counters;
   uint32_t* counters_host;
   uint32_t counter_words;
-};
+  uint32_t flags;
+  uint32_t* regbits_n;
+};
+#define ZES_PAR_NO_REGBITS 1u
 
 struct ZesSegRes {
   uint64_t end_bit;
@@ -192,7 +195,7 @@
 __global__ void k_inf_first_bytes(const uint8_t*, const uint64_t*, uint8_t*, uint32_t);
 __global__ void k_inf_scan(const uint8_t*, const ZesInfBuf*, uint32_t, unsigned long long*, uint32_t, uint32_t*, uint8_t*, uint32_t,
                            const uint8_t*);
-__global__ void k_inf_set_table1(ZesInfBuf, ZesInfBuf, ZesInfBuf*, uint32_t*, uint32_t);
+__global__ void k_inf_set_table1(ZesInfBuf, ZesInfBuf, ZesInfBuf*, uint32_t*, uint32_t, uint32_t*);
 __global__ void k_inf_verify(const uint8_t*, const ZesInfBuf*, const unsigned long long*, uint32_t, uint32_t*, uint32_t*, uint32_t*, uint32_t, uint32_t*, uint32_t, uint32_t);
 __global__ void k_inf_verify_long(const uint8_t*, const ZesInfBuf*, const unsigned long long*, uint32_t, uint32_t*, uint32_t*, uint32_t*, uint32_t, const uint32_t*, uint32_t);
 __global__ void k_inf_ranksort(const ZesInfBuf*, const uint32_t*, const uint32_t*, uint32_t*, uint32_t);
```

Result: slower. 44.28 GiB/s (-2.9%).
